# Thefefe/orbit

Hardware: AMD Instinct MI355X
Metric: meshlets_culled_per_sec (higher is better)
Workload: dtype f32

## Files before the change

### bindings/rust/orbit_hip.rs

```rust
#![allow(non_camel_case_types, dead_code)]
use std::ffi::{c_char, c_void};

#[repr(C)]
pub struct OrbitCtx { _private: [u8; 0] }
#[repr(C)]
pub struct OrbitMeshletStream { _private: [u8; 0] }

#[repr(C)] #[derive(Clone, Copy, Default)]
pub struct OrbitCaps {
    pub max_entities: u32, pub max_dispatches: u32, pub max_draws: u32, pub max_lights: u32,
    pub max_clusters: u32, pub dispatch_size: u32, pub max_views: u32, pub validate_streams: u32, pub cull_path: u32,
    pub arith_profile: u32,
}

#[repr(C)]
pub struct OrbitClusterFrame {
    pub push: *const c_void, pub info: *const c_void, pub depth: *const f32, pub lights: *const c_void,
    pub tile_depth_slice_mask: *mut u32, pub depth_bounds: *mut c_void, pub unique_cluster_buffer: *mut c_void,
    pub light_index_buffer: *mut c_void, pub cluster_offset_image: *mut u32,
    pub index_capacity: u32, pub light_index_capacity: u32,
}
#[repr(C)]
pub struct OrbitFrameLate {
    pub pyramids: *const c_void, pub late_views: *const c_void, pub cascade_views: *const c_void,
// ... 162 lines not shown
                                   draw_first: u32, draw_count: u32, stream: *mut c_void) -> i32;
    pub fn orbit_meshlet_cull(ctx: *mut OrbitCtx, cull_info: *const c_void, bufs: *const OrbitMeshletCullBufs,
                              stream: *mut c_void) -> i32;
    pub fn orbit_depth_pyramid_desc(screen_w: u32, screen_h: u32, desc: *mut OrbitDepthPyramidDesc) -> i32;
    pub fn orbit_depth_pyramid_desc_from_mip0(mip0_w: u32, mip0_h: u32, desc: *mut OrbitDepthPyramidDesc) -> i32;
    pub fn orbit_ctx_profile(ctx: *mut OrbitCtx, enable: i32) -> i32;
    pub fn orbit_ctx_profile_reserve(ctx: *mut OrbitCtx, pairs: u32, stream: *mut c_void) -> i32;
    pub fn orbit_ctx_profile_read(ctx: *mut OrbitCtx, avg_ms: *mut f32, launches: *mut u32) -> i32;
    pub fn orbit_cull_views(ctx: *mut OrbitCtx, views: *const OrbitCullView, count: u32, stream: *mut c_void) -> i32;
    pub fn orbit_depth_reduce(ctx: *mut OrbitCtx, depth: *const f32, screen_w: u32, screen_h: u32,
                              pyramid: *mut f32, stream: *mut c_void) -> i32;
    pub fn orbit_depth_reduce_multi(ctx: *mut OrbitCtx, items: *const OrbitDepthReduceItem, count: u32,
                                    stream: *mut c_void) -> i32;
    pub fn orbit_cluster_mark(ctx: *mut OrbitCtx, push: *const c_void, depth: *const f32, masks: *mut u32,
                              bounds: *mut c_void, stream: *mut c_void) -> i32;
    pub fn orbit_cluster_compact(ctx: *mut OrbitCtx, cluster_count: *const [u32; 3], masks: *const u32,
                                 unique: *mut c_void, index_capacity: u32, stream: *mut c_void) -> i32;
    pub fn orbit_cluster_assign(ctx: *mut OrbitCtx, info: *const c_void, unique: *const c_void, bounds: *const c_void,
                                lights: *const c_void, light_index_buffer: *mut c_void, light_index_capacity: u32,
                                cluster_offset_image: *mut u32, stream: *mut c_void) -> i32;
    pub fn orbit_meshlet_task_cull(ctx: *mut OrbitCtx, cull_info: *const c_void, bufs: *const c_void,
                                   task_records: *mut c_void, stream: *mut c_void) -> i32;
    pub fn orbit_compute_clusters(ctx: *mut OrbitCtx, push: *const c_void, info: *const c_void, depth: *const f32,
                                  lights: *const c_void, masks: *mut u32, bounds: *mut c_void, unique: *mut c_void,
                                  index_capacity: u32, light_index_buffer: *mut c_void, light_index_capacity: u32,
                                  cluster_offset_image: *mut u32, stream: *mut c_void) -> i32;
    pub fn orbit_shard_range(entity_draw_count: u32, rank: u32, world: u32, begin: *mut u32, end: *mut u32);
    pub fn orbit_gather_visible(ctx: *mut OrbitCtx, nccl_comm: *mut c_void, rank: u32, world: u32,
                                local_draw_buffer: *const c_void, out_draw_buffer: *mut c_void, out_capacity: u32,
                                stream: *mut c_void) -> i32;
    pub fn orbit_meshlet_cull_visible_records(ctx: *mut OrbitCtx, cull_info: *const c_void, bufs: *const c_void,
                                              record_buffer: *mut c_void, record_capacity: u32,
                                              stream: *mut c_void) -> i32;
    pub fn orbit_expand_visible_records(ctx: *mut OrbitCtx, record_buffer: *const c_void, meshlet_buffer: *const c_void,
                                        draw_commands_buffer: *mut c_void, draw_capacity: u32,
                                        stream: *mut c_void) -> i32;
    pub fn orbit_meshlet_stream_create(ctx: *mut OrbitCtx, first_meshlet: u64, capacity: u64,
                                       out_stream: *mut *mut OrbitMeshletStream) -> i32;
    pub fn orbit_meshlet_stream_update(ctx: *mut OrbitCtx, ms: *mut OrbitMeshletStream, meshlet_buffer: *const c_void,
                                       first: u64, count: u64, stream: *mut c_void) -> i32;
    pub fn orbit_meshlet_stream_set_materials(ctx: *mut OrbitCtx, ms: *mut OrbitMeshletStream, material_buffer: *const c_void,
                                              material_count: u32, stream: *mut c_void) -> i32;
    pub fn orbit_meshlet_stream_validate(ctx: *mut OrbitCtx, ms: *mut OrbitMeshletStream, meshlet_buffer: *const c_void,
                                         material_buffer: *const c_void, stream: *mut c_void) -> i32;
    pub fn orbit_meshlet_stream_destroy(ms: *mut OrbitMeshletStream) -> i32;
    pub fn orbit_meshlet_stream_update_meshes(ctx: *mut OrbitCtx, ms: *mut OrbitMeshletStream, mesh_info_buffer: *const c_void,
                                              first_mesh: u32, count: u32, stream: *mut c_void) -> i32;
    pub fn orbit_ctx_mesh_side_culls(ctx: *const OrbitCtx) -> u64;
    pub fn orbit_ctx_bind_meshlet_stream(ctx: *mut OrbitCtx, ms: *mut OrbitMeshletStream) -> i32;
    pub fn orbit_ctx_fused_culls(ctx: *const OrbitCtx) -> u64;
    pub fn orbit_frame_late(ctx: *mut OrbitCtx, frame: *const OrbitFrameLate, stream: *mut c_void) -> i32;
    pub fn orbit_ctx_meshlet_stream_culls(ctx: *const OrbitCtx) -> u64;
    pub fn orbit_ctx_meshlet_class_culls(ctx: *const OrbitCtx) -> u64;
    pub fn orbit_p2p_alloc(ctx: *mut OrbitCtx, bytes: u64, out_ptr: *mut *mut c_void, out_handle: *mut [u8; 64]) -> i32;
    pub fn orbit_p2p_free(ctx: *mut OrbitCtx, ptr: *mut c_void) -> i32;
    pub fn orbit_p2p_open(ctx: *mut OrbitCtx, handle: *const [u8; 64], out_peer_ptr: *mut *mut c_void) -> i32;
    pub fn orbit_p2p_close(ctx: *mut OrbitCtx, peer_ptr: *mut c_void) -> i32;
    pub fn orbit_meshlet_cull_records_and_commands(ctx: *mut OrbitCtx, cull_info: *const c_void,
                                                   bufs: *const OrbitMeshletCullBufs, record_buffer: *mut c_void,
                                                   record_capacity: u32, stream: *mut c_void) -> i32;
    pub fn orbit_exchange_list(ctx: *mut OrbitCtx, local_list: *const c_void, rank: u32, world: u32,
                               out_buffers: *const *mut c_void, ctrl_buffers: *const *mut c_void, out_capacity: u32,
                               header_bytes: u32, stride: u32, stream: *mut c_void) -> i32;
    pub fn orbit_cull_shard(ctx: *mut OrbitCtx, cull_info: *const c_void, entity_bufs: *const OrbitEntityCullBufs,
                            draw_first: u32, draw_count: u32, meshlet_bufs: *const OrbitMeshletCullBufs,
                            record_buffer: *mut c_void, record_capacity: u32, with_commands: u32,
                            stream: *mut c_void) -> i32;
    pub fn orbit_ctx_shard_culls(ctx: *const OrbitCtx) -> u64;
    pub fn orbit_allgather_list(ctx: *mut OrbitCtx, nccl_comm: *mut c_void, rank: u32, world: u32,
                                local_list: *const c_void, segment_capacity: u32, segments: *mut c_void,
                                out_list: *mut c_void, out_capacity: u32, header_bytes: u32, stride: u32,
                                stream: *mut c_void) -> i32;
    pub fn orbit_compact_segments(ctx: *mut OrbitCtx, segments: *const c_void, world: u32, segment_capacity: u32,
                                  out_list: *mut c_void, out_capacity: u32, header_bytes: u32, stride: u32,
                                  stream: *mut c_void) -> i32;
    pub fn orbit_scene_update_entities(ctx: *mut OrbitCtx, transforms: *const OrbitEntityTransform,
                                       instance_indices: *const u32, count: u32, entity_data: *mut c_void,
                                       entity_capacity: u32, stream: *mut c_void) -> i32;
    pub fn orbit_scene_update(ctx: *mut OrbitCtx, update: *const OrbitSceneUpdate, stream: *mut c_void) -> i32;
    pub fn orbit_cull_stats(ctx: *mut OrbitCtx, cull_info: *const c_void, ebufs: *const OrbitEntityCullBufs,
                            entity_draw_count: u32, mbufs: *const OrbitMeshletCullBufs, stats: *mut OrbitCullStats,
                            stream: *mut c_void) -> i32;
    pub fn orbit_cluster_stats(ctx: *mut OrbitCtx, push: *const c_void, info: *const c_void, depth: *const f32,
                               lights: *const c_void, stats: *mut OrbitClusterStats, stream: *mut c_void) -> i32;
    pub fn orbit_meshlet_bounds(ctx: *mut OrbitCtx, job: *const OrbitMeshletBoundsJob, stream: *mut c_void) -> i32;
    pub fn orbit_mesh_bounds(ctx: *mut OrbitCtx, ranges: *const OrbitMeshBoundsRange, range_count: u32,
                             vertices: *const c_void, vertex_count: u64, vertex_stride: u32, position_offset: u32,
                             mesh_infos: *mut c_void, mesh_capacity: u32, stream: *mut c_void) -> i32;
    pub fn orbit_raster_depth(ctx: *mut OrbitCtx, job: *const OrbitRasterDepth, stream: *mut c_void) -> i32;
    pub fn orbit_raster_visibility(ctx: *mut OrbitCtx, job: *const OrbitRasterVisibility, stream: *mut c_void) -> i32;
    pub fn orbit_visibility_resolve(ctx: *mut OrbitCtx, job: *const OrbitVisibilityResolve, stream: *mut c_void) -> i32;
}

pub fn check(ctx: *const OrbitCtx, rc: i32) {
    if rc != 0 {
        let msg = unsafe { std::ffi::CStr::from_ptr(orbit_last_error(ctx)) }.to_string_lossy().into_owned();
        panic!("orbit_hip error {rc}: {msg}");
    }
}
```

### include/orbit_abi_ext.h

```cpp
#ifndef ORBIT_ABI_EXT_H
#define ORBIT_ABI_EXT_H

#include "orbit_abi.h"

#ifdef __cplusplus
extern "C" {
#endif

#define ORBIT_VISIBLE_HEADER 8u
typedef struct OrbitVisibleRecord {
    uint32_t entity_index;
    uint32_t meshlet_offset;
    uint32_t mask;
} OrbitVisibleRecord;
ORBIT_STATIC_ASSERT(sizeof(OrbitVisibleRecord) == 12, "visible record is 12 B");

int32_t orbit_meshlet_task_cull(OrbitCtx *ctx, const OrbitGpuCullInfo *cull_info,
                                const OrbitMeshletCullBufs *bufs,
                                OrbitMeshTaskRecord *task_records, void *stream);

typedef struct OrbitCullView {
    const OrbitGpuCullInfo *cull_info;
    OrbitEntityCullBufs entity;
    OrbitMeshletCullBufs meshlet;
    uint32_t entity_draw_count;
    uint32_t skip_meshlet_stage;
} OrbitCullView;
#define ORBIT_MAX_CULL_VIEWS 8
int32_t orbit_cull_views(OrbitCtx *ctx, const OrbitCullView *views, uint32_t count, void *stream);
uint64_t orbit_ctx_fused_culls(const OrbitCtx *ctx);

typedef struct OrbitMeshletStream OrbitMeshletStream;
int32_t orbit_meshlet_stream_create(OrbitCtx *ctx, uint64_t first_meshlet, uint64_t capacity,
                                    OrbitMeshletStream **out_stream);
int32_t orbit_meshlet_stream_update(OrbitCtx *ctx, OrbitMeshletStream *ms, const void *meshlet_buffer,
                                    uint64_t first, uint64_t count, void *stream);
int32_t orbit_meshlet_stream_set_materials(OrbitCtx *ctx, OrbitMeshletStream *ms, const void *material_buffer,
                                           uint32_t material_count, void *stream);
int32_t orbit_meshlet_stream_validate(OrbitCtx *ctx, OrbitMeshletStream *ms, const void *meshlet_buffer,
                                      const void *material_buffer, void *stream);
int32_t orbit_meshlet_stream_update_meshes(OrbitCtx *ctx, OrbitMeshletStream *ms, const void *mesh_info_buffer,
                                           uint32_t first_mesh, uint32_t count, void *stream);
uint64_t orbit_ctx_mesh_side_culls(const OrbitCtx *ctx);
int32_t orbit_meshlet_stream_destroy(OrbitMeshletStream *ms);
int32_t orbit_ctx_bind_meshlet_stream(OrbitCtx *ctx, OrbitMeshletStream *ms);
uint64_t orbit_ctx_meshlet_stream_culls(const OrbitCtx *ctx);
uint64_t orbit_ctx_meshlet_class_culls(const OrbitCtx *ctx);

typedef struct OrbitDepthReduceItem {
    const float *depth;
    uint32_t screen_width, screen_height;
    uint32_t depth_row_pitch;
    uint32_t _pad;
    float *pyramid;
    const OrbitDepthPyramidLevel *levels;
} OrbitDepthReduceItem;
ORBIT_STATIC_ASSERT(sizeof(OrbitDepthReduceItem) == 40, "depth-reduce item is 40 B");
#define ORBIT_MAX_PYRAMID_BATCH 8
int32_t orbit_depth_reduce_multi(OrbitCtx *ctx, const OrbitDepthReduceItem *items, uint32_t count, void *stream);

typedef struct OrbitClusterFrame {
    const OrbitMarkActivePush *push;
    const OrbitClusterCullInfo *info;
    const float *depth;
    const OrbitLightData *lights;
    uint32_t *tile_depth_slice_mask;
    OrbitClusterDepthBounds *depth_bounds;
    void *unique_cluster_buffer;
    void *light_index_buffer;
    uint32_t *cluster_offset_image;
    uint32_t index_capacity;
    uint32_t light_index_capacity;
} OrbitClusterFrame;
ORBIT_STATIC_ASSERT(sizeof(OrbitClusterFrame) == 80, "cluster frame block is 80 B");
typedef struct OrbitFrameLate {
    const OrbitDepthReduceItem *pyramids;
    const OrbitCullView *late_views;
    const OrbitCullView *cascade_views;
    const OrbitClusterFrame *clusters;
    uint32_t pyramid_count, late_view_count, cascade_view_count, _pad;
} OrbitFrameLate;
ORBIT_STATIC_ASSERT(sizeof(OrbitFrameLate) == 48, "frame-late descriptor is 48 B");
int32_t orbit_frame_late(OrbitCtx *ctx, const OrbitFrameLate *frame, void *stream);

int32_t orbit_ctx_profile(OrbitCtx *ctx, int32_t enable);
int32_t orbit_ctx_profile_reserve(OrbitCtx *ctx, uint32_t pairs, void *stream);
int32_t orbit_ctx_profile_read(OrbitCtx *ctx, float *avg_ms, uint32_t *launches);

int32_t orbit_meshlet_cull_visible_records(OrbitCtx *ctx, const OrbitGpuCullInfo *cull_info,
                                           const OrbitMeshletCullBufs *bufs, void *record_buffer,
                                           uint32_t record_capacity, void *stream);
int32_t orbit_expand_visible_records(OrbitCtx *ctx, const void *record_buffer, const void *meshlet_buffer,
                                     void *draw_commands_buffer, uint32_t draw_capacity, void *stream);
int32_t orbit_meshlet_cull_records_and_commands(OrbitCtx *ctx, const OrbitGpuCullInfo *cull_info,
                                                const OrbitMeshletCullBufs *bufs, void *record_buffer,
                                                uint32_t record_capacity, void *stream);
int32_t orbit_cull_shard(OrbitCtx *ctx, const OrbitGpuCullInfo *cull_info, const OrbitEntityCullBufs *entity_bufs,
                         uint32_t draw_first, uint32_t draw_count, const OrbitMeshletCullBufs *meshlet_bufs,
                         void *record_buffer, uint32_t record_capacity, uint32_t with_commands, void *stream);
uint64_t orbit_ctx_shard_culls(const OrbitCtx *ctx);
// ... 228 lines not shown
```

### orbit_amd/_lib.py

```python
import ctypes as C
import os

_HERE = os.path.dirname(os.path.abspath(__file__))
LIB_PATH = os.path.join(_HERE, "liborbit_cull.so")

OK, E_INVALID, E_PLANES, E_CAPACITY, E_HIP, E_NO_DEVICE, E_TIMEOUT, E_MISSING, E_COMM, E_RANGE, E_STALE = (
    0, -1, -2, -3, -4, -5, -6, -7, -8, -9, -10)
ERROR_NAMES = {
    E_INVALID: "ORBIT_E_INVALID", E_PLANES: "ORBIT_E_PLANES", E_CAPACITY: "ORBIT_E_CAPACITY", E_HIP: "ORBIT_E_HIP",
    E_NO_DEVICE: "ORBIT_E_NO_DEVICE", E_TIMEOUT: "ORBIT_E_TIMEOUT", E_MISSING: "ORBIT_E_MISSING",
    E_COMM: "ORBIT_E_COMM", E_RANGE: "ORBIT_E_RANGE", E_STALE: "ORBIT_E_STALE",
}

MAX_PYRAMID_MIPS = 16


class OrbitError(RuntimeError):
    def __init__(self, code, message):
        super().__init__(f"{ERROR_NAMES.get(code, code)}: {message}")
        self.code = code


class Caps(C.Structure):
    _fields_ = [("max_entities", C.c_uint32), ("max_dispatches", C.c_uint32), ("max_draws", C.c_uint32),
# ... 104 lines not shown
                                                            C.c_void_p, C.c_uint32, C.c_void_p]),
    "orbit_exchange_list": (C.c_int32, [C.c_void_p, C.c_void_p, C.c_uint32, C.c_uint32, C.POINTER(C.c_void_p),
                                        C.POINTER(C.c_void_p), C.c_uint32, C.c_uint32, C.c_uint32, C.c_void_p]),
    "orbit_ctx_fused_culls": (C.c_uint64, [C.c_void_p]),
    "orbit_frame_late": (C.c_int32, [C.c_void_p, C.POINTER(FrameLate), C.c_void_p]),
    "orbit_default_caps": (None, [C.POINTER(Caps)]),
    "orbit_ctx_create": (C.c_int32, [C.c_int32, C.POINTER(Caps), C.POINTER(C.c_void_p)]),
    "orbit_ctx_destroy": (C.c_int32, [C.c_void_p]),
    "orbit_last_error": (C.c_char_p, [C.c_void_p]),
    "orbit_ctx_status": (C.c_int32, [C.c_void_p, C.c_void_p, C.c_int32]),
    "orbit_entity_cull": (C.c_int32, [C.c_void_p, C.c_void_p, C.POINTER(EntityCullBufs), C.c_uint32, C.c_void_p]),
    "orbit_entity_cull_range": (C.c_int32, [C.c_void_p, C.c_void_p, C.POINTER(EntityCullBufs), C.c_uint32,
                                            C.c_uint32, C.c_void_p]),
    "orbit_meshlet_cull": (C.c_int32, [C.c_void_p, C.c_void_p, C.POINTER(MeshletCullBufs), C.c_void_p]),
    "orbit_meshlet_task_cull": (C.c_int32, [C.c_void_p, C.c_void_p, C.POINTER(MeshletCullBufs), C.c_void_p, C.c_void_p]),
    "orbit_depth_pyramid_desc": (C.c_int32, [C.c_uint32, C.c_uint32, C.POINTER(DepthPyramidDesc)]),
    "orbit_cull_views": (C.c_int32, [C.c_void_p, C.POINTER(CullView), C.c_uint32, C.c_void_p]),
    "orbit_depth_reduce_multi": (C.c_int32, [C.c_void_p, C.POINTER(DepthReduceItem), C.c_uint32, C.c_void_p]),
    "orbit_depth_pyramid_desc_from_mip0": (C.c_int32, [C.c_uint32, C.c_uint32, C.POINTER(DepthPyramidDesc)]),
    "orbit_depth_reduce": (C.c_int32, [C.c_void_p, C.c_void_p, C.c_uint32, C.c_uint32, C.c_void_p, C.c_void_p]),
    "orbit_cluster_mark": (C.c_int32, [C.c_void_p, C.c_void_p, C.c_void_p, C.c_void_p, C.c_void_p, C.c_void_p]),
    "orbit_cluster_compact": (C.c_int32, [C.c_void_p, C.POINTER(C.c_uint32 * 3), C.c_void_p, C.c_void_p, C.c_uint32,
                                          C.c_void_p]),
    "orbit_cluster_assign": (C.c_int32, [C.c_void_p, C.c_void_p, C.c_void_p, C.c_void_p, C.c_void_p, C.c_void_p,
                                         C.c_uint32, C.c_void_p, C.c_void_p]),
    "orbit_compute_clusters": (C.c_int32, [C.c_void_p, C.c_void_p, C.c_void_p, C.c_void_p, C.c_void_p, C.c_void_p,
                                           C.c_void_p, C.c_void_p, C.c_uint32, C.c_void_p, C.c_uint32, C.c_void_p,
                                           C.c_void_p]),
    "orbit_ctx_profile": (C.c_int32, [C.c_void_p, C.c_int32]),
    "orbit_ctx_profile_reserve": (C.c_int32, [C.c_void_p, C.c_uint32, C.c_void_p]),
    "orbit_ctx_profile_read": (C.c_int32, [C.c_void_p, C.POINTER(C.c_float), C.POINTER(C.c_uint32)]),
    "orbit_shard_range": (None, [C.c_uint32, C.c_uint32, C.c_uint32, C.POINTER(C.c_uint32), C.POINTER(C.c_uint32)]),
    "orbit_gather_visible": (C.c_int32, [C.c_void_p, C.c_void_p, C.c_uint32, C.c_uint32, C.c_void_p, C.c_void_p,
                                         C.c_uint32, C.c_void_p]),
    "orbit_meshlet_cull_visible_records": (C.c_int32, [C.c_void_p, C.c_void_p, C.POINTER(MeshletCullBufs), C.c_void_p,
                                                       C.c_uint32, C.c_void_p]),
    "orbit_expand_visible_records": (C.c_int32, [C.c_void_p, C.c_void_p, C.c_void_p, C.c_void_p, C.c_uint32,
                                                 C.c_void_p]),
    "orbit_p2p_alloc": (C.c_int32, [C.c_void_p, C.c_uint64, C.POINTER(C.c_void_p), C.c_void_p]),
    "orbit_p2p_free": (C.c_int32, [C.c_void_p, C.c_void_p]),
    "orbit_p2p_open": (C.c_int32, [C.c_void_p, C.c_void_p, C.POINTER(C.c_void_p)]),
    "orbit_p2p_close": (C.c_int32, [C.c_void_p, C.c_void_p]),
    "orbit_meshlet_stream_create": (C.c_int32, [C.c_void_p, C.c_uint64, C.c_uint64, C.POINTER(C.c_void_p)]),
    "orbit_meshlet_stream_update": (C.c_int32, [C.c_void_p, C.c_void_p, C.c_void_p, C.c_uint64, C.c_uint64,
                                                C.c_void_p]),
    "orbit_meshlet_stream_set_materials": (C.c_int32, [C.c_void_p, C.c_void_p, C.c_void_p, C.c_uint32, C.c_void_p]),
    "orbit_meshlet_stream_validate": (C.c_int32, [C.c_void_p, C.c_void_p, C.c_void_p, C.c_void_p, C.c_void_p]),
    "orbit_meshlet_stream_destroy": (C.c_int32, [C.c_void_p]),
    "orbit_meshlet_stream_update_meshes": (C.c_int32, [C.c_void_p, C.c_void_p, C.c_void_p, C.c_uint32, C.c_uint32, C.c_void_p]),
    "orbit_ctx_mesh_side_culls": (C.c_uint64, [C.c_void_p]),
    "orbit_ctx_bind_meshlet_stream": (C.c_int32, [C.c_void_p, C.c_void_p]),
    "orbit_ctx_meshlet_stream_culls": (C.c_uint64, [C.c_void_p]),
    "orbit_ctx_meshlet_class_culls": (C.c_uint64, [C.c_void_p]),
    "orbit_cull_shard": (C.c_int32, [C.c_void_p, C.c_void_p, C.POINTER(EntityCullBufs), C.c_uint32, C.c_uint32,
                                     C.POINTER(MeshletCullBufs), C.c_void_p, C.c_uint32, C.c_uint32, C.c_void_p]),
    "orbit_ctx_shard_culls": (C.c_uint64, [C.c_void_p]),
    "orbit_allgather_list": (C.c_int32, [C.c_void_p, C.c_void_p, C.c_uint32, C.c_uint32, C.c_void_p, C.c_uint32,
                                         C.c_void_p, C.c_void_p, C.c_uint32, C.c_uint32, C.c_uint32, C.c_void_p]),
    "orbit_compact_segments": (C.c_int32, [C.c_void_p, C.c_void_p, C.c_uint32, C.c_uint32, C.c_void_p, C.c_uint32,
                                           C.c_uint32, C.c_uint32, C.c_void_p]),
    "orbit_scene_update_entities": (C.c_int32, [C.c_void_p, C.c_void_p, C.c_void_p, C.c_uint32, C.c_void_p, C.c_uint32,
                                                C.c_void_p]),
    "orbit_scene_update": (C.c_int32, [C.c_void_p, C.POINTER(SceneUpdate), C.c_void_p]),
    "orbit_cull_stats": (C.c_int32, [C.c_void_p, C.c_void_p, C.POINTER(EntityCullBufs), C.c_uint32,
                                     C.POINTER(MeshletCullBufs), C.c_void_p, C.c_void_p]),
    "orbit_cluster_stats": (C.c_int32, [C.c_void_p, C.c_void_p, C.c_void_p, C.c_void_p, C.c_void_p, C.c_void_p,
                                        C.c_void_p]),
    "orbit_meshlet_bounds": (C.c_int32, [C.c_void_p, C.POINTER(MeshletBoundsJob), C.c_void_p]),
    "orbit_mesh_bounds": (C.c_int32, [C.c_void_p, C.c_void_p, C.c_uint32, C.c_void_p, C.c_uint64, C.c_uint32, C.c_uint32,
                                      C.c_void_p, C.c_uint32, C.c_void_p]),
    "orbit_raster_depth": (C.c_int32, [C.c_void_p, C.POINTER(RasterDepth), C.c_void_p]),
    "orbit_raster_visibility": (C.c_int32, [C.c_void_p, C.POINTER(RasterVisibility), C.c_void_p]),
    "orbit_visibility_resolve": (C.c_int32, [C.c_void_p, C.POINTER(VisibilityResolve), C.c_void_p]),
}

_lib = None


def load_variant(path):
    import torch

    lib = C.CDLL(path)
    for name, (restype, argtypes) in SYMBOLS.items():
        if hasattr(lib, name):
            fn = getattr(lib, name)
            fn.restype = restype
            fn.argtypes = argtypes
    return lib


def load():
    global _lib
    if _lib is not None:
        return _lib
    if not os.path.exists(LIB_PATH):
        raise OSError(f"{LIB_PATH} is missing: build it with `make -C orbit_amd/csrc` or "
                      "`python -c 'import __graft_entry__ as g; g.build()'` (there is no fallback path)")
    try:
        import torch
    except ImportError:
        pass
    lib = C.CDLL(LIB_PATH)
    for name, (restype, argtypes) in SYMBOLS.items():
        fn = getattr(lib, name)
        fn.restype = restype
        fn.argtypes = argtypes
# ... 9 lines not shown
```

### orbit_amd/csrc/abi_ctx.hip

```cpp
#include <cstdarg>
#include <cstdio>
#include <cstdlib>

#include "abi_internal.h"

thread_local char g_err[512] = "no error";

int32_t fail(OrbitCtx *ctx, int32_t code, const char *fmt, ...) {
    char buf[512];
    va_list ap;
    va_start(ap, fmt);
    vsnprintf(buf, sizeof(buf), fmt, ap);
    va_end(ap);
    snprintf(g_err, sizeof(g_err), "%s", buf);
    if (ctx) snprintf(ctx->err, sizeof(ctx->err), "%s", buf);
    return code;
}

namespace {

size_t layout_arena(OrbitCtx *ctx, uintptr_t base, uint64_t md32) {
    const OrbitCaps &caps = ctx->caps;
    const size_t ent = align_up((size_t)caps.max_entities, 256);
    const size_t mtiles = ((size_t)md32 + kTileRecords - 1) / kTileRecords + 1;
// ... 84 lines not shown
                    caps.max_dispatches, caps.dispatch_size, max_dispatch_capacity());
    if (caps.arith_profile > ORBIT_ARITH_CONTRACTED)
        return fail(nullptr, ORBIT_E_INVALID, "arith_profile %u (0 canonical, 1 contracted)", caps.arith_profile);
    if (caps.max_dispatches > max_dispatch_capacity())
        return fail(nullptr, ORBIT_E_CAPACITY, "caps.max_dispatches %u > %u (chunk-base table of the emit launch)",
                    caps.max_dispatches, max_dispatch_capacity());
    int ndev = 0;
    hipError_t e = hipGetDeviceCount(&ndev);
    if (e != hipSuccess || ndev <= 0 || device_id < 0 || device_id >= ndev)
        return fail(nullptr, ORBIT_E_NO_DEVICE, "no usable HIP device %d (count %d): %s; there is no CPU fallback",
                    device_id, ndev, e == hipSuccess ? "ok" : hipGetErrorString(e));
    hipDeviceProp_t prop;
    e = hipGetDeviceProperties(&prop, device_id);
    if (e != hipSuccess) return hip_fail(nullptr, e, "hipGetDeviceProperties");
    if (strncmp(prop.gcnArchName, "gfx950", 6) != 0)
        return fail(nullptr, ORBIT_E_NO_DEVICE, "device %d is %s; this library carries gfx950 code objects only",
                    device_id, prop.gcnArchName);
    e = hipSetDevice(device_id);
    if (e != hipSuccess) return hip_fail(nullptr, e, "hipSetDevice");
    if (caps.cull_path > 2u)
        return fail(nullptr, ORBIT_E_INVALID, "caps.cull_path %u (0 auto, 1 launch chain, 2 one-launch cull)", caps.cull_path);
    if (caps.max_views > ORBIT_MAX_CULL_VIEWS)
        return fail(nullptr, ORBIT_E_CAPACITY, "caps.max_views %u > %u", caps.max_views, (unsigned)ORBIT_MAX_CULL_VIEWS);

    OrbitCtx *ctx = new (std::nothrow) OrbitCtx();
    if (!ctx) return fail(nullptr, ORBIT_E_HIP, "out of host memory");
    ctx->device = device_id;
    ctx->num_cus = (uint32_t)prop.multiProcessorCount;
    for (uint32_t v = 0; v < kRasterVariants; v++)
        with_raster_variant((RasterVariant)v, [&](auto variant) {
            ctx->raster_blocks[v] = ctx->num_cus * raster_depth_blocks_per_cu<variant.value>();
            ctx->visibility_blocks[v] = ctx->num_cus * raster_visibility_blocks_per_cu<variant.value>();
        });
    ctx->caps = caps;
    ctx->rec_shift = rec_shift;

    ctx->arena_bytes = layout_arena(ctx, 0, md32);
    e = hipMalloc((void **)&ctx->arena, ctx->arena_bytes);
    if (e != hipSuccess) {
        delete ctx;
        return hip_fail(nullptr, e, "hipMalloc(scratch arena)");
    }
    e = memset_now(ctx->arena, 0, ctx->arena_bytes);
    if (e != hipSuccess) {
        (void)hipFree(ctx->arena);
        delete ctx;
        return hip_fail(nullptr, e, "hipMemset(scratch arena)");
    }
    (void)layout_arena(ctx, (uintptr_t)ctx->arena, md32);
#ifdef ORBIT_TRIAGE
    const char *dbg = getenv("ORBIT_SP_DEBUG");
    ctx->debug_flags = dbg ? (uint32_t)atoi(dbg) : 0u;
#endif
    snprintf(ctx->err, sizeof(ctx->err), "no error");
    const OrbitCaps child_caps = view_child_caps(caps);
    for (uint32_t v = 1; v < caps.max_views; v++) {
        OrbitCtx *child = nullptr;
        const int32_t rc = orbit_ctx_create(device_id, &child_caps, &child);
        if (rc != ORBIT_OK) {
            (void)orbit_ctx_destroy(ctx);
            return rc;
        }
        ctx->view_ctx.push_back(child);
    }
    *out_ctx = ctx;
    return ORBIT_OK;
}

int32_t orbit_ctx_destroy(OrbitCtx *ctx) {
    if (!ctx) return ORBIT_OK;
    (void)hipSetDevice(ctx->device);
    (void)hipDeviceSynchronize();
    for (hipEvent_t ev : ctx->prof_events) (void)hipEventDestroy(ev);
    for (hipEvent_t ev : ctx->side_event)
        if (ev) (void)hipEventDestroy(ev);
    for (hipStream_t st : ctx->side_stream)
        if (st) (void)hipStreamDestroy(st);
    for (OrbitCtx *child : ctx->view_ctx) (void)orbit_ctx_destroy(child);
    if (ctx->meshlet_stream) ctx->meshlet_stream->bindings.fetch_sub(1);
    if (ctx->arena) (void)hipFree(ctx->arena);
    delete ctx;
    return ORBIT_OK;
}

int32_t orbit_ctx_status(OrbitCtx *ctx, void *stream, int32_t sync) {
    if (!ctx) return fail(nullptr, ORBIT_E_INVALID, "ctx is NULL");
    std::lock_guard<std::mutex> lock(ctx->mu);
    hipStream_t s = (hipStream_t)stream;
    if (sync) {
        hipError_t e = hipStreamSynchronize(s);
        if (e != hipSuccess) return hip_fail(ctx, e, "hipStreamSynchronize");
    }
    int32_t v = 0;
    hipError_t e = hipMemcpy(&v, ctx->status, 4, hipMemcpyDeviceToHost);
    if (e != hipSuccess) return hip_fail(ctx, e, "hipMemcpy(status)");
    for (OrbitCtx *child : ctx->view_ctx) {
        int32_t cv = 0;
        e = hipMemcpy(&cv, child->status, 4, hipMemcpyDeviceToHost);
        if (e != hipSuccess) return hip_fail(ctx, e, "hipMemcpy(status)");
        if (cv != 0) {
            (void)memset_now(child->status, 0, 4);
            if (v == 0) v = cv;
        }
    }
    if (v != 0) {
        e = memset_now(ctx->status, 0, 4);
// ... 117 lines not shown
```

### orbit_amd/csrc/abi_cull.hip

```cpp
#include "abi_internal.h"

namespace {

int32_t check_cull_info(OrbitCtx *ctx, const OrbitGpuCullInfo *ci) {
    if (!ci) return fail(ctx, ORBIT_E_INVALID, "cull_info is NULL");
    if (ci->cull_plane_count > ORBIT_MAX_CULL_PLANES)
        return fail(ctx, ORBIT_E_PLANES, "cull_plane_count %u > %d", ci->cull_plane_count, ORBIT_MAX_CULL_PLANES);
    if (ci->projection_type > 1) return fail(ctx, ORBIT_E_INVALID, "projection_type %u", ci->projection_type);
    if (ci->occlusion_pass > 2) return fail(ctx, ORBIT_E_INVALID, "occlusion_pass %u", ci->occlusion_pass);
    return ORBIT_OK;
}

MeshSideView mesh_side_for(OrbitMeshletStream *ms, const void *mesh_info_buffer, bool count = true) {
    if (!ms) return MeshSideView{nullptr, 0u};
    std::lock_guard<std::mutex> lock(ms->mu);
    if (ms->mesh_side == nullptr || ms->mesh_source != mesh_info_buffer || ms->mesh_hi == 0u) return MeshSideView{nullptr, 0u};
    if (count) ms->mesh_side_culls++;
    return MeshSideView{ms->mesh_side, ms->mesh_hi};
}

PyramidView make_pyramid_view(const float *texels, const uint32_t size[2],
                              const OrbitDepthPyramidLevel *levels = nullptr) {
    PyramidView v;
    v.texels = texels;
// ... 131 lines not shown
        ok = ok && zero(pl[4][0]) && zero(pl[4][1]);
        const float v[6] = {pl[0][0], pl[0][2], pl[2][1], pl[2][2], pl[4][2], pl[4][3]};
        for (float f : v) ok = ok && fin(f);
        p.std_planes = ok ? 1u : 0u;
        for (int k = 0; k < 6; k++) p.stdp[k] = ok ? v[k] : 0.0f;
    }
    p.task_records = task ? (OrbitMeshTaskRecord *)out.buffer : nullptr;
    p.also_commands = out.also_commands ? (uint8_t *)b->draw_commands_buffer : nullptr;
    p.also_commands_capacity = out.also_commands ? b->draw_capacity : 0u;
    p.tile_counts = scratch->m_tile_counts;
    p.tile_masks = scratch->m_tile_masks;
    p.tile_payload = scratch->m_tile_payload;
    p.tile_base = scratch->m_tile_base;
    p.chunk_sums = scratch->m_chunk_sums;
    p.total = scratch->m_total;
    p.tickets = scratch->m_tickets;
    p.list_sync = scratch->m_list_sync;
    p.debug_flags = scratch->debug_flags;
    p.debug_cycles = scratch->debug_cycles;
    p.scan_patience = ctx->scan_patience;
    p.zero_page = scratch->zero_page;
    p.status = scratch->status;
    return ORBIT_OK;
}

SplitRecordsParams split_params_for(const OrbitCtx *ctx, const OrbitCtx *scratch, const OrbitMeshletCullBufs *b) {
    SplitRecordsParams sp;
    sp.src = (const uint8_t *)b->meshlet_dispatch_buffer;
    sp.dst = scratch->m_split;
    sp.src_capacity = b->dispatch_capacity;
    sp.rec_shift = ctx->rec_shift;
    return sp;
}

int32_t profile_pair(OrbitCtx *ctx, hipEvent_t &ev0, hipEvent_t &ev1) {
    ev0 = ev1 = nullptr;
    if (!ctx->profiling || (ctx->prof_calls++ % ctx->profiling) != 0) return ORBIT_OK;
    if (ctx->prof_used + 2 > ctx->prof_events.size()) {
        for (int i = 0; i < 2; i++) {
            hipEvent_t ev;
            if (hipEventCreate(&ev) != hipSuccess) return fail(ctx, ORBIT_E_HIP, "hipEventCreate");
            ctx->prof_events.push_back(ev);
        }
    }
    ev0 = ctx->prof_events[ctx->prof_used];
    ev1 = ctx->prof_events[ctx->prof_used + 1];
    ctx->prof_used += 2;
    return ORBIT_OK;
}

int32_t validate_stream(OrbitCtx *ctx, const MeshletCullParams &p, hipStream_t s) {
    if (!p.ms.sphere || !ctx->caps.validate_streams) return ORBIT_OK;
    const hipError_t e = launch_meshlet_stream_validate(p.meshlets, p.ms, p.ms.cls0 ? p.materials : nullptr,
                                                        ctx->meshlet_stream->material_count, ctx->status, s);
    return e == hipSuccess ? ORBIT_OK : hip_fail(ctx, e, "launch meshlet_stream_validate");
}

void count_stream_cull(OrbitCtx *ctx, const MeshletCullParams &p) {
    if (p.ms.sphere && p.ci.occlusion_pass != 1) {
        ctx->stream_culls++;
        if (p.ms.cls0) ctx->class_culls++;
    }
}

int32_t entity_cull_impl(OrbitCtx *ctx, const OrbitGpuCullInfo *ci, const OrbitEntityCullBufs *b, uint32_t draw_first,
                         uint32_t entity_draw_count, bool exact_range, void *stream) {
    if (!ctx) return fail(nullptr, ORBIT_E_INVALID, "ctx is NULL");
    std::lock_guard<std::mutex> lock(ctx->mu);
    EntityCullParams p;
    int32_t rc = entity_cull_params(ctx, ctx, ci, b, draw_first, entity_draw_count, exact_range, p);
    if (rc == ORBIT_OK) rc = validate_mesh_side(ctx, p, (hipStream_t)stream);
    if (rc) return rc;
    const hipError_t e = launch_entity_cull(p, entity_draw_count, ctx->num_cus, (hipStream_t)stream);
    if (e != hipSuccess) return hip_fail(ctx, e, "launch entity_cull");
    return ORBIT_OK;
}

int32_t meshlet_cull_impl(OrbitCtx *ctx, const OrbitGpuCullInfo *ci, const OrbitMeshletCullBufs *b,
                          const MeshletCullOut &out, void *stream) {
    if (!ctx) return fail(nullptr, ORBIT_E_INVALID, "ctx is NULL");
    std::lock_guard<std::mutex> lock(ctx->mu);
    const hipStream_t s = (hipStream_t)stream;
    MeshletCullParams p;
    hipEvent_t ev0, ev1;
    int32_t rc = meshlet_cull_params(ctx, ctx, ci, b, out, p);
    if (rc == ORBIT_OK) rc = profile_pair(ctx, ev0, ev1);
    if (rc == ORBIT_OK && ci->occlusion_pass != 1) rc = validate_stream(ctx, p, s);
    if (rc) return rc;
    hipError_t e = hipSuccess;
    if (ctx->rec_shift > 5u) e = launch_split_records(split_params_for(ctx, ctx, b), s);
    if (e != hipSuccess) return hip_fail(ctx, e, "launch split_records");
    e = launch_meshlet_cull(p, ctx->num_cus, s, ev0, ev1);
    if (e != hipSuccess) return hip_fail(ctx, e, "launch meshlet_cull");
    count_stream_cull(ctx, p);
    return ORBIT_OK;
}

FusedCullParams fused_params(const EntityCullParams &ep, const MeshletCullParams &mp, const OrbitCtx *scratch,
                             uint32_t chunks) {
    FusedCullParams f{};
    f.m = mp;
    f.entity_draw_buffer = ep.entity_draw_buffer;
    f.mesh_infos = ep.mesh_infos;
    f.mesh_side = ep.mesh_side;
    f.visibility = ep.visibility;
    f.e_pyr = ep.pyr;
    f.draw_first = ep.draw_first;
    f.draw_limit = ep.draw_limit;
    f.e_dispatch_capacity = ep.dispatch_capacity;
    f.ne_chunks = chunks;
    f.e_total = ep.total;
    f.sync = scratch->f_sync;
    f.ent_flags = scratch->f_ent_flags;
    f.tile_flags = scratch->f_tile_flags;
    return f;
}

OrbitCtx *scratch_of(OrbitCtx *ctx, uint32_t k) { return k == 0 ? ctx : ctx->view_ctx[k - 1]; }

}

int32_t prepare_cull_views(OrbitCtx *ctx, const OrbitCullView *views, uint32_t count, uint32_t scratch_base,
                           PreparedCullViews &pc) {
    if (!views || count == 0) return fail(ctx, ORBIT_E_MISSING, "cull_views: no views");
    if (count > ORBIT_MAX_CULL_VIEWS || scratch_base + count > ORBIT_MAX_CULL_VIEWS)
        return fail(ctx, ORBIT_E_CAPACITY, "cull_views: %u views (max %u)", scratch_base + count, (unsigned)ORBIT_MAX_CULL_VIEWS);
    hipError_t e = hipSetDevice(ctx->device);
    if (e != hipSuccess) return hip_fail(ctx, e, "hipSetDevice");
    while (ctx->view_ctx.size() + 1 < scratch_base + count) {
        OrbitCtx *child = nullptr;
        const OrbitCaps child_caps = view_child_caps(ctx->caps);
        const int32_t rc = orbit_ctx_create(ctx->device, &child_caps, &child);
        if (rc != ORBIT_OK) return fail(ctx, rc, "cull_views: scratch for view %zu: %s", ctx->view_ctx.size() + 1, g_err);
        ctx->view_ctx.push_back(child);
    }
    pc.count = count;
    for (uint32_t i = 0; i < count; i++) {
        const OrbitCullView &v = views[i];
        OrbitCtx *scratch = scratch_of(ctx, scratch_base + i);
        int32_t rc = entity_cull_params(ctx, scratch, v.cull_info, &v.entity, 0u, v.entity_draw_count, false, pc.ev.v[i]);
        if (rc == ORBIT_OK && !v.skip_meshlet_stage) {
            rc = meshlet_cull_params(ctx, scratch, v.cull_info, &v.meshlet, MeshletCullOut{}, pc.mv.v[pc.n_mesh]);
            if (rc == ORBIT_OK && ctx->rec_shift > 5u) pc.sv.v[pc.n_mesh] = split_params_for(ctx, scratch, &v.meshlet);
            if (rc == ORBIT_OK && v.meshlet.meshlet_dispatch_buffer != v.entity.meshlet_dispatch_buffer)
                rc = fail(ctx, ORBIT_E_INVALID, "view %u: the meshlet stage must read the entity stage's dispatch buffer", i);
            pc.n_mesh++;
        }
// ... 209 lines not shown
```

### orbit_amd/csrc/abi_internal.h

```cpp
#pragma once
#include <hip/hip_runtime.h>

#include <atomic>
#include <cstdint>
#include <cstring>
#include <mutex>
#include <new>
#include <vector>

#include "kernels.h"

using namespace orbit;

#pragma GCC visibility push(hidden)

struct OrbitMeshletStream {
    int device = 0;
    uint64_t first = 0, capacity = 0;
    uint4 *sphere = nullptr;
    uint32_t *cone = nullptr;
    uint16_t *mat = nullptr;
    uint32_t *cmd = nullptr;
    uint16_t *cnt = nullptr;
    uint32_t *link = nullptr, *cls0 = nullptr, *cls1 = nullptr;
    uint2 *base32 = nullptr;
    std::mutex mu;
    const void *source = nullptr;
    uint64_t valid_lo = 0, valid_hi = 0;
    const void *materials = nullptr;
    uint32_t material_count = 0;
    uint32_t *d_other = nullptr, *h_other = nullptr;
    hipEvent_t other_event = nullptr;
    bool other_pending = false;
    bool other_recorded = false;
    std::atomic<int> bindings{0};
    MeshSide *mesh_side = nullptr;
    uint32_t mesh_capacity = 0, mesh_hi = 0;
    const void *mesh_source = nullptr;
    uint64_t mesh_side_culls = 0;
};

struct OrbitCtx {
    int device = 0;
    uint32_t num_cus = 0;
    OrbitCaps caps{};
    std::mutex mu;
    uint8_t *arena = nullptr;
    size_t arena_bytes = 0;
    OrbitMeshletDispatch *e_proto = nullptr;
    uint32_t *e_block_sums = nullptr, *e_total = nullptr;
    Payload *m_tile_payload = nullptr;
    uint32_t *m_tile_masks = nullptr, *m_chunk_sums = nullptr;
    uint32_t *m_tile_counts = nullptr, *m_tile_base = nullptr, *m_total = nullptr;
    uint32_t *s_block_sums = nullptr;
    uint32_t raster_blocks[kRasterVariants] = {};
    uint32_t visibility_blocks[kRasterVariants] = {};
    float *b_mesh_slices = nullptr;
    uint32_t *x_block_pop = nullptr;
    uint32_t *c_chunk = nullptr;
    size_t c_chunk_words = 0;
    float4 *a_view_lights = nullptr, *a_coarse_lights = nullptr;
    uint32_t *a_light_flags = nullptr, *a_counts = nullptr, *a_block_sums = nullptr, *a_block_base = nullptr,
             *a_total = nullptr, *a_coarse = nullptr, *a_coarse_counts = nullptr, *a_hit_cache = nullptr;
    float *a_aabb = nullptr, *a_group_box = nullptr;
    uint32_t *a_group_order = nullptr;
    uint32_t a_coarse_seg = 0;
    uint32_t *m_tickets = nullptr, *m_list_sync = nullptr, *f_done = nullptr;
    uint32_t *f_sync = nullptr, *f_ent_flags = nullptr, *f_tile_flags = nullptr;
    uint32_t *d_tickets = nullptr;
    uint8_t *m_split = nullptr;
    uint32_t rec_shift = 5;
    uint64_t fused_culls = 0;
    uint64_t shard_culls = 0;
    uint32_t *g_counts = nullptr;
    int32_t *status = nullptr;
    uint32_t debug_flags = 0;
    uint32_t scan_patience = 256;
    unsigned long long *debug_cycles = nullptr;
    void *zero_page = nullptr;
    uint32_t profiling = 0;
    uint32_t prof_calls = 0;
    std::vector<hipEvent_t> prof_events;
    size_t prof_used = 0;
    std::vector<OrbitCtx *> view_ctx;
    hipStream_t side_stream[2] = {nullptr, nullptr};
    hipEvent_t side_event[3] = {nullptr, nullptr, nullptr};
    OrbitMeshletStream *meshlet_stream = nullptr;
    uint64_t stream_culls = 0;
    uint64_t class_culls = 0;
    char err[512] = {0};
};

constexpr uint32_t kExpandBlocks = 65536;

constexpr uint32_t kMeshBoundsSlots = 1024;

extern thread_local char g_err[512];

int32_t fail(OrbitCtx *ctx, int32_t code, const char *fmt, ...);

inline int32_t hip_fail(OrbitCtx *ctx, hipError_t e, const char *what) {
    return fail(ctx, ORBIT_E_HIP, "%s: %s", what, hipGetErrorString(e));
}

inline size_t align_up(size_t v, size_t a) { return (v + a - 1) / a * a; }

inline hipError_t memset_now(void *ptr, int value, size_t bytes) {
    hipError_t e = hipMemset(ptr, value, bytes);
    if (e == hipSuccess) e = hipStreamSynchronize(nullptr);
    return e;
}

inline uint32_t mip_levels_from_size(uint32_t max_size) {
    uint32_t l = 0;
    while ((max_size >> (l + 1)) != 0) l++;
    return l + 1;
}

inline OrbitCaps view_child_caps(OrbitCaps child_caps) {
    child_caps.max_views = 0, child_caps.max_clusters = 0, child_caps.max_lights = 0;
    return child_caps;
}

inline MeshletStreamView stream_arrays(const OrbitMeshletStream *ms, uint64_t lo, uint64_t hi) {
    MeshletStreamView v{};
    v.sphere = ms->sphere - ms->first;
    v.cone = ms->cone - ms->first;
    v.mat = ms->mat - ms->first;
    v.cmd = ms->cmd - 3u * ms->first;
    v.cnt = ms->cnt - ms->first;
    v.link = ms->link - (ms->first >> 5);
    v.base32 = ms->base32 - (ms->first >> 5);
    v.cls0 = ms->cls0 - (ms->first >> 5);
    v.cls1 = ms->cls1 - (ms->first >> 5);
    v.first = (uint32_t)lo;
    v.count = (uint32_t)(hi - lo);
    return v;
}

inline MeshletStreamView stream_view_for(OrbitMeshletStream *ms, const void *meshlet_buffer, const void *material_buffer) {
    if (!ms) return MeshletStreamView{};
    std::lock_guard<std::mutex> lock(ms->mu);
    if (ms->source == nullptr || ms->source != meshlet_buffer || ms->valid_hi == ms->valid_lo) return MeshletStreamView{};
    MeshletStreamView v = stream_arrays(ms, ms->valid_lo, ms->valid_hi);
    bool classes = ms->materials != nullptr && ms->materials == material_buffer;
    if (classes && ms->other_pending && ms->other_recorded && hipEventQuery(ms->other_event) == hipSuccess)
        ms->other_pending = false;
    if (classes && (ms->other_pending || *ms->h_other != 0u)) classes = false;
    if (!classes) v.cls0 = v.cls1 = nullptr;
    return v;
}

struct PreparedCullViews {
    EntityCullViews ev{};
    MeshletCullViews mv{};
    FusedCullViews fv{};
    SplitRecordsViews sv{};
    uint32_t draws[ORBIT_MAX_CULL_VIEWS] = {};
    uint32_t count = 0, n_mesh = 0, max_draws = 0;
    bool fused = false;
};

int32_t prepare_cull_views(OrbitCtx *ctx, const OrbitCullView *views, uint32_t count, uint32_t scratch_base,
                           PreparedCullViews &pc);
int32_t launch_prepared_cull_views(OrbitCtx *ctx, const PreparedCullViews &pc, hipStream_t s);

#pragma GCC visibility pop
```

### orbit_amd/csrc/abi_stream.hip

```cpp
#include "abi_internal.h"

namespace {

constexpr uint32_t kMeshSideMinCapacity = 1u << 20;

hipError_t read_back_class_flag(OrbitMeshletStream *ms, hipStream_t s) {
    ms->other_pending = true;
    ms->other_recorded = false;
    hipStreamCaptureStatus cs = hipStreamCaptureStatusNone;
    if (hipStreamIsCapturing(s, &cs) != hipSuccess || cs != hipStreamCaptureStatusNone) return hipSuccess;
    hipError_t e = hipMemcpyAsync(ms->h_other, ms->d_other, sizeof(uint32_t), hipMemcpyDeviceToHost, s);
    if (e == hipSuccess) e = hipEventRecord(ms->other_event, s);
    if (e == hipSuccess) ms->other_recorded = true;
    return e;
}

int32_t check_stream(OrbitCtx *ctx, const OrbitMeshletStream *ms, const char *who, bool takes_buffer = false, const void *buffer = nullptr) {
    if (takes_buffer ? !ms || !buffer : !ms)
        return fail(ctx, ORBIT_E_MISSING, takes_buffer ? "%s: NULL argument" : "%s: stream is NULL", who);
    if (ms->device != ctx->device) return fail(ctx, ORBIT_E_INVALID, "%s: stream lives on device %d", who, ms->device);
    return ORBIT_OK;
}

}

extern "C" {

int32_t orbit_meshlet_stream_create(OrbitCtx *ctx, uint64_t first_meshlet, uint64_t capacity,
                                    OrbitMeshletStream **out_stream) {
    if (!ctx) return fail(nullptr, ORBIT_E_INVALID, "ctx is NULL");
    std::lock_guard<std::mutex> lock(ctx->mu);
    if (!out_stream) return fail(ctx, ORBIT_E_MISSING, "meshlet_stream_create: out_stream is NULL");
    *out_stream = nullptr;
    if (capacity == 0 || capacity > (1ull << 27) || first_meshlet + capacity > 0xFFFFFFFFull)
        return fail(ctx, ORBIT_E_INVALID, "meshlet_stream_create: range [%llu, +%llu) (at most 2^27 meshlets per stream)",
                    (unsigned long long)first_meshlet, (unsigned long long)capacity);
    hipError_t e = hipSetDevice(ctx->device);
    if (e != hipSuccess) return hip_fail(ctx, e, "hipSetDevice");
    OrbitMeshletStream *ms = new (std::nothrow) OrbitMeshletStream();
    if (!ms) return fail(ctx, ORBIT_E_HIP, "out of host memory");
    ms->device = ctx->device;
    ms->first = first_meshlet;
    ms->capacity = capacity;
    const size_t bit_words = (size_t)(((first_meshlet + capacity + 31u) >> 5) - (first_meshlet >> 5)) + 2u;
    struct {
        void **p;
        size_t bytes;
        int fill;
    } arrays[] = {{(void **)&ms->sphere, capacity * sizeof(uint4), 0},
                  {(void **)&ms->cone, capacity * sizeof(uint32_t), 0},
                  {(void **)&ms->mat, capacity * sizeof(uint16_t) + 256u, 0},
                  {(void **)&ms->cmd, capacity * 12u, 0},
                  {(void **)&ms->cnt, capacity * sizeof(uint16_t) + 256u, 0},
                  {(void **)&ms->link, bit_words * sizeof(uint32_t), 0},
                  {(void **)&ms->base32, bit_words * sizeof(uint2), 0},
                  {(void **)&ms->cls0, bit_words * sizeof(uint32_t), 0xFF},
                  {(void **)&ms->cls1, bit_words * sizeof(uint32_t), 0xFF}};
    for (auto &a : arrays) {
        if (e == hipSuccess) e = hipMalloc(a.p, a.bytes);
        if (e == hipSuccess) e = hipMemset(*a.p, a.fill, a.bytes);
    }
    if (e == hipSuccess) e = hipMalloc((void **)&ms->d_other, 256);
    if (e == hipSuccess) e = memset_now(ms->d_other, 0, 256);
    if (e == hipSuccess) e = hipHostMalloc((void **)&ms->h_other, sizeof(uint32_t), hipHostMallocDefault);
    if (e == hipSuccess) *ms->h_other = 0u;
    if (e == hipSuccess) e = hipEventCreateWithFlags(&ms->other_event, hipEventDisableTiming);
    if (e != hipSuccess) {
        orbit_meshlet_stream_destroy(ms);
        return hip_fail(ctx, e, "meshlet_stream_create: hipMalloc (36.65 B per meshlet)");
    }
    *out_stream = ms;
    return ORBIT_OK;
}

int32_t orbit_meshlet_stream_update(OrbitCtx *ctx, OrbitMeshletStream *ms, const void *meshlet_buffer, uint64_t first,
                                    uint64_t count, void *stream) {
    if (!ctx) return fail(nullptr, ORBIT_E_INVALID, "ctx is NULL");
    std::lock_guard<std::mutex> lock(ctx->mu);
    if (const int32_t rc = check_stream(ctx, ms, "meshlet_stream_update", true, meshlet_buffer)) return rc;
    if (first < ms->first || count > ms->capacity || first - ms->first > ms->capacity - count)
        return fail(ctx, ORBIT_E_CAPACITY, "meshlet_stream_update: [%llu, +%llu) outside the stream's [%llu, +%llu)",
                    (unsigned long long)first, (unsigned long long)count, (unsigned long long)ms->first,
                    (unsigned long long)ms->capacity);
    std::lock_guard<std::mutex> slock(ms->mu);
    const bool same = ms->source == meshlet_buffer && ms->valid_hi > ms->valid_lo;
    const uint64_t lo = same ? (first < ms->valid_lo ? first : ms->valid_lo) : first;
    const uint64_t hi = same ? (first + count > ms->valid_hi ? first + count : ms->valid_hi) : first + count;
    MeshletStreamView v = stream_arrays(ms, same ? ms->valid_lo : first, same ? ms->valid_hi : first + count);
    if (v.first > first) v.count += v.first - (uint32_t)first, v.first = (uint32_t)first;
    if ((uint64_t)v.first + v.count < first + count) v.count = (uint32_t)(first + count - v.first);
    hipError_t e = launch_meshlet_stream_build((const OrbitMeshlet *)meshlet_buffer, first, count, v,
                                               (const OrbitMaterialData *)ms->materials, ms->material_count, ms->d_other,
                                               (hipStream_t)stream);
    if (e != hipSuccess) return hip_fail(ctx, e, "launch meshlet_stream_build");
    if (ms->materials != nullptr && count != 0) {
        e = read_back_class_flag(ms, (hipStream_t)stream);
        if (e != hipSuccess) return hip_fail(ctx, e, "meshlet_stream_update: class flag read-back");
    }
    if (count != 0) {
        ms->source = meshlet_buffer;
        ms->valid_lo = lo;
        ms->valid_hi = hi;
    }
    return ORBIT_OK;
}

int32_t orbit_meshlet_stream_set_materials(OrbitCtx *ctx, OrbitMeshletStream *ms, const void *material_buffer,
                                           uint32_t material_count, void *stream) {
    if (!ctx) return fail(nullptr, ORBIT_E_INVALID, "ctx is NULL");
    std::unique_lock<std::mutex> lock(ctx->mu);
    if (const int32_t rc = check_stream(ctx, ms, "meshlet_stream_set_materials")) return rc;
    if (material_buffer && material_count == 0)
        return fail(ctx, ORBIT_E_INVALID, "meshlet_stream_set_materials: material_count is 0");
    std::unique_lock<std::mutex> slock(ms->mu);
    ms->other_pending = true;
    ms->other_recorded = false;
    hipError_t e = hipMemsetAsync(ms->d_other, 0, sizeof(uint32_t), (hipStream_t)stream);
    if (e == hipSuccess)
        e = launch_meshlet_stream_classes(stream_arrays(ms, ms->first, ms->first + ms->capacity),
                                          (const OrbitMaterialData *)material_buffer, material_buffer ? material_count : 0u,
                                          ms->d_other, (hipStream_t)stream);
    if (e == hipSuccess) e = read_back_class_flag(ms, (hipStream_t)stream);
    if (e != hipSuccess) return hip_fail(ctx, e, "launch meshlet_stream_classes");
    ms->materials = material_buffer;
    ms->material_count = material_buffer ? material_count : 0u;
    const bool wait = ms->other_recorded;
    hipEvent_t ev = ms->other_event;
    slock.unlock();
    lock.unlock();
    if (wait) {
        e = hipEventSynchronize(ev);
        if (e != hipSuccess) {
            lock.lock();
            return hip_fail(ctx, e, "hipEventSynchronize(alpha-class flag)");
        }
    }
    return ORBIT_OK;
}

int32_t orbit_meshlet_stream_update_meshes(OrbitCtx *ctx, OrbitMeshletStream *ms, const void *mesh_info_buffer,
                                           uint32_t first_mesh, uint32_t count, void *stream) {
    if (!ctx) return fail(nullptr, ORBIT_E_INVALID, "ctx is NULL");
    std::lock_guard<std::mutex> lock(ctx->mu);
    if (const int32_t rc = check_stream(ctx, ms, "meshlet_stream_update_meshes")) return rc;
    std::lock_guard<std::mutex> slock(ms->mu);
    if (!mesh_info_buffer) {
        ms->mesh_source = nullptr;
// ... 9 lines not shown
        if (e == hipSuccess) e = memset_now(ms->mesh_side, 0, (size_t)cap * sizeof(MeshSide));
        if (e != hipSuccess) {
            (void)hipFree(ms->mesh_side);
            ms->mesh_side = nullptr;
            return hip_fail(ctx, e, "meshlet_stream_update_meshes: hipMalloc (32 B per mesh)");
        }
        ms->mesh_capacity = cap;
    }
    if (first_mesh + count > ms->mesh_capacity)
        return fail(ctx, ORBIT_E_CAPACITY, "meshlet_stream_update_meshes: meshes [%u, +%u) beyond the table's %u", first_mesh,
                    count, ms->mesh_capacity);
    if (ms->mesh_source != mesh_info_buffer && ms->mesh_hi != 0u) {
        e = hipMemsetAsync(ms->mesh_side, 0, (size_t)ms->mesh_hi * sizeof(MeshSide), (hipStream_t)stream);
        if (e != hipSuccess) return hip_fail(ctx, e, "meshlet_stream_update_meshes: hipMemsetAsync");
        ms->mesh_hi = 0u;
    }
    e = launch_mesh_side_build((const OrbitMeshInfo *)mesh_info_buffer, first_mesh, count, ms->mesh_side, (hipStream_t)stream);
    if (e != hipSuccess) return hip_fail(ctx, e, "launch mesh_side_build");
    if (count != 0u) {
        ms->mesh_source = mesh_info_buffer;
        if (first_mesh + count > ms->mesh_hi) ms->mesh_hi = first_mesh + count;
    }
    return ORBIT_OK;
}

uint64_t orbit_ctx_mesh_side_culls(const OrbitCtx *ctx) {
    if (!ctx || !ctx->meshlet_stream) return 0;
    std::lock_guard<std::mutex> lock(ctx->meshlet_stream->mu);
    return ctx->meshlet_stream->mesh_side_culls;
}

int32_t orbit_meshlet_stream_validate(OrbitCtx *ctx, OrbitMeshletStream *ms, const void *meshlet_buffer,
                                      const void *material_buffer, void *stream) {
    if (!ctx) return fail(nullptr, ORBIT_E_INVALID, "ctx is NULL");
    std::lock_guard<std::mutex> lock(ctx->mu);
    if (const int32_t rc = check_stream(ctx, ms, "meshlet_stream_validate", true, meshlet_buffer)) return rc;
    {
        std::lock_guard<std::mutex> slock(ms->mu);
        if (ms->mesh_side != nullptr && ms->mesh_source != nullptr && ms->mesh_hi != 0u) {
            const hipError_t me = launch_mesh_side_validate((const OrbitMeshInfo *)ms->mesh_source, 0u, ms->mesh_hi, ms->mesh_side,
                                                            ctx->status, (hipStream_t)stream);
            if (me != hipSuccess) return hip_fail(ctx, me, "launch mesh_side_validate");
        }
    }
    MeshletStreamView v = stream_view_for(ms, meshlet_buffer, nullptr);
    if (!v.sphere) return ORBIT_OK;
    const bool classes = material_buffer != nullptr && ms->materials == material_buffer;
    if (classes) {
        const MeshletStreamView all = stream_arrays(ms, ms->first, ms->first + ms->capacity);
        v.cls0 = all.cls0, v.cls1 = all.cls1;
    }
    const hipError_t e = launch_meshlet_stream_validate((const OrbitMeshlet *)meshlet_buffer, v,
                                                        classes ? (const OrbitMaterialData *)material_buffer : nullptr,
                                                        ms->material_count, ctx->status, (hipStream_t)stream);
    if (e != hipSuccess) return hip_fail(ctx, e, "launch meshlet_stream_validate");
    return ORBIT_OK;
}

int32_t orbit_meshlet_stream_destroy(OrbitMeshletStream *ms) {
    if (!ms) return ORBIT_OK;
    if (ms->bindings.load() > 0)
        return fail(nullptr, ORBIT_E_INVALID, "meshlet_stream_destroy: the stream is still bound to %d context(s)",
                    ms->bindings.load());
    (void)hipFree(ms->sphere);
    (void)hipFree(ms->cone);
    (void)hipFree(ms->mat);
    (void)hipFree(ms->cmd);
    (void)hipFree(ms->cnt);
    (void)hipFree(ms->link);
    (void)hipFree(ms->base32);
    (void)hipFree(ms->cls0);
    (void)hipFree(ms->cls1);
    (void)hipFree(ms->d_other);
    (void)hipFree(ms->mesh_side);
    if (ms->h_other) (void)hipHostFree(ms->h_other);
    if (ms->other_event) (void)hipEventDestroy(ms->other_event);
    delete ms;
    return ORBIT_OK;
}

int32_t orbit_ctx_bind_meshlet_stream(OrbitCtx *ctx, OrbitMeshletStream *ms) {
    if (!ctx) return fail(nullptr, ORBIT_E_INVALID, "ctx is NULL");
    std::lock_guard<std::mutex> lock(ctx->mu);
    if (const int32_t rc = ms ? check_stream(ctx, ms, "bind_meshlet_stream") : ORBIT_OK) return rc;
    if (ms) ms->bindings.fetch_add(1);
    if (ctx->meshlet_stream) ctx->meshlet_stream->bindings.fetch_sub(1);
    ctx->meshlet_stream = ms;
    return ORBIT_OK;
}

uint64_t orbit_ctx_fused_culls(const OrbitCtx *ctx) { return ctx ? ctx->fused_culls : 0; }
uint64_t orbit_ctx_meshlet_stream_culls(const OrbitCtx *ctx) { return ctx ? ctx->stream_culls : 0; }
uint64_t orbit_ctx_meshlet_class_culls(const OrbitCtx *ctx) { return ctx ? ctx->class_culls : 0; }
uint64_t orbit_ctx_shard_culls(const OrbitCtx *ctx) { return ctx ? ctx->shard_culls : 0; }

}
```

### orbit_amd/csrc/kernels.h

```cpp
#pragma once
#include <hip/hip_runtime.h>
#include <stdint.h>
#include <type_traits>

#include "../../include/orbit_abi_ext.h"
#include "orbit_device.h"

namespace orbit {

constexpr uint32_t kTileRecords = 16;
constexpr uint32_t kTileRows = 8;
constexpr uint32_t kTicketPools = 8;
constexpr uint32_t kTicketStride = 64;
constexpr uint32_t kEmitTicketPools = 16;
constexpr uint32_t kListGroups = 32;
constexpr uint32_t kListSyncStride = 32;
constexpr uint32_t kListSyncWords = (kListGroups + 1) * kListSyncStride;

struct Payload {
    uint32_t y, z, w;
};

struct MeshSide {
    float sphere[4];
    uint32_t lod_count, lod0_offset, lod0_count, valid;
};
static_assert(sizeof(MeshSide) == 32, "MeshSide layout");
struct MeshSideView {
    const MeshSide *table;
    uint32_t count;
};

struct EntityCullParams {
    OrbitGpuCullInfo ci;
    const uint8_t *entity_draw_buffer;
    const OrbitMeshInfo *mesh_infos;
    MeshSideView mesh_side;
    uint8_t *dispatch_buffer;
    const OrbitEntityData *entities;
    uint32_t *visibility;
    PyramidView pyr;
    uint32_t draw_first;
    uint32_t draw_limit;
    uint32_t dispatch_capacity;
    uint32_t ne_chunks;
    uint32_t rec_shift;
    uint32_t arith;
    OrbitMeshletDispatch *proto;
    uint32_t *block_sums;
    uint32_t *sync;
    uint32_t *ent_flags;
    uint32_t *total;
    int32_t *status;
};

struct MeshletStreamView {
    const uint4 *sphere;
    const uint32_t *cone;
    const uint16_t *mat;
    const uint32_t *cmd;
    const uint16_t *cnt;
// ... 121 lines not shown
    PyramidView e_pyr;
    uint32_t draw_first, draw_limit;
    uint32_t e_dispatch_capacity;
    uint32_t ne_chunks;
    uint32_t *e_total;
    uint32_t *sync;
    uint32_t *ent_flags;
    uint32_t *tile_flags;
    uint32_t *done_flags;
};
struct FusedCullViews {
    FusedCullParams v[ORBIT_MAX_CULL_VIEWS];
};
hipError_t launch_cull_fused_views(const FusedCullViews &all, const uint32_t *entity_draw_counts, uint32_t n,
                                   uint32_t num_cus, hipStream_t s);
constexpr uint32_t kShardMaxChunks = 256;
constexpr uint32_t kShardDoneWords = 64, kShardDoneStride = 32;
hipError_t launch_shard_cull(const FusedCullParams &f, uint32_t num_cus, hipStream_t s);
hipError_t launch_meshlet_scan_emit(const MeshletCullParams &p, uint32_t num_cus, hipStream_t s);

hipError_t launch_entity_cull(const EntityCullParams &p, uint32_t entity_draw_count, uint32_t num_cus, hipStream_t s);
struct SplitRecordsParams {
    const uint8_t *src;
    uint8_t *dst;
    uint32_t src_capacity;
    uint32_t rec_shift;
};
struct SplitRecordsViews {
    SplitRecordsParams v[ORBIT_MAX_CULL_VIEWS];
};
hipError_t launch_split_records(const SplitRecordsParams &p, hipStream_t s);
hipError_t launch_split_records_views(const SplitRecordsViews &all, uint32_t n, hipStream_t s);

struct EntityCullViews {
    EntityCullParams v[ORBIT_MAX_CULL_VIEWS];
};
struct MeshletCullViews;
struct FusedCullViews;
struct ViewGroup;
#if !ORBIT_CONTRACT
hipError_t launch_entity_cull_contracted(const EntityCullParams &p, uint32_t entity_draw_count, uint32_t num_cus, hipStream_t s);
hipError_t launch_entity_cull_views_contracted(const EntityCullViews &all, uint32_t n, uint32_t max_entity_draw_count,
                                               uint32_t num_cus, hipStream_t s);
hipError_t launch_meshlet_eval_contracted(const MeshletCullParams &p, uint32_t num_cus, hipStream_t s);
hipError_t launch_meshlet_eval_views_contracted(const MeshletCullViews &all, const ViewGroup &g, uint32_t m, uint32_t pass,
                                                bool ortho, int src, uint32_t max_tiles, uint32_t num_cus, hipStream_t s);
hipError_t launch_shard_cull_contracted(const FusedCullParams &f, uint32_t num_cus, hipStream_t s);
hipError_t launch_cull_fused_views_contracted(const FusedCullViews &all, const uint32_t *entity_draw_counts, uint32_t n,
                                              uint32_t num_cus, hipStream_t s);
#endif
hipError_t launch_entity_cull_views(const EntityCullViews &all, uint32_t n, uint32_t max_entity_draw_count,
                                    uint32_t num_cus, hipStream_t s);
hipError_t launch_meshlet_cull(const MeshletCullParams &p, uint32_t num_cus, hipStream_t s,
                               hipEvent_t ev0 = nullptr, hipEvent_t ev1 = nullptr);
struct MeshletCullViews {
    MeshletCullParams v[ORBIT_MAX_CULL_VIEWS];
};
hipError_t launch_meshlet_cull_views(const MeshletCullViews &all, uint32_t n, uint32_t num_cus, hipStream_t s);
struct ViewGroup {
    uint8_t idx[ORBIT_MAX_CULL_VIEWS];
};
hipError_t launch_meshlet_eval(const MeshletCullParams &p, uint32_t num_cus, hipStream_t s);
hipError_t launch_meshlet_eval_views(const MeshletCullViews &all, const ViewGroup &g, uint32_t m, uint32_t pass,
                                     bool ortho, int src, uint32_t max_tiles, uint32_t num_cus, hipStream_t s);
hipError_t launch_meshlet_emit(const MeshletCullParams &p, bool stream, uint32_t num_cus, hipStream_t s);
hipError_t launch_meshlet_emit_views(const MeshletCullViews &all, const ViewGroup &g, uint32_t m, uint32_t n, bool stream,
                                     uint32_t max_tiles_all, uint32_t num_cus, hipStream_t s);
hipError_t launch_task_records(const MeshletCullParams &p, hipStream_t s);
uint32_t max_dispatch_capacity();
hipError_t launch_meshlet_stream_build(const OrbitMeshlet *meshlets, uint64_t first, uint64_t count,
                                       const MeshletStreamView &ms, const OrbitMaterialData *materials,
                                       uint32_t material_count, uint32_t *other, hipStream_t s);
hipError_t launch_meshlet_stream_validate(const OrbitMeshlet *meshlets, const MeshletStreamView &ms,
                                          const OrbitMaterialData *materials, uint32_t material_count, int32_t *status,
                                          hipStream_t s);
hipError_t launch_scene_update_entities(const OrbitEntityTransform *transforms, const uint32_t *instance_indices,
                                        uint32_t count, OrbitEntityData *entity_data, uint32_t entity_capacity,
                                        int32_t *status, hipStream_t s);
hipError_t launch_scene_update(const OrbitSceneUpdate &u, uint32_t *block_sums, int32_t *status, hipStream_t s);
hipError_t launch_meshlet_bounds(const OrbitMeshletBoundsJob &job, uint32_t num_cus, int32_t *status, hipStream_t s);
hipError_t launch_mesh_bounds(const OrbitMeshBoundsRange *ranges, uint32_t range_count, uint32_t slices,
                              const void *vertices, uint64_t vertex_count, uint32_t vertex_stride,
                              uint32_t position_offset, OrbitMeshInfo *mesh_infos, uint32_t mesh_capacity, float *scratch,
                              int32_t *status, hipStream_t s);
enum class RasterVariant : uint32_t { Plain, ClipNear, Wide };
constexpr uint32_t kRasterVariants = 3;
inline RasterVariant raster_variant(uint32_t flags) {
    return (flags & ORBIT_RASTER_WIDE_GUARD) ? RasterVariant::Wide : (flags & ORBIT_RASTER_CLIP_NEAR) ? RasterVariant::ClipNear : RasterVariant::Plain;
}
template <class F>
inline auto with_raster_variant(RasterVariant v, F f) {
    switch (v) {
    case RasterVariant::Wide: return f(std::integral_constant<RasterVariant, RasterVariant::Wide>{});
    case RasterVariant::ClipNear: return f(std::integral_constant<RasterVariant, RasterVariant::ClipNear>{});
    default: return f(std::integral_constant<RasterVariant, RasterVariant::Plain>{});
    }
}
template <RasterVariant V>
hipError_t launch_raster_depth(const OrbitRasterDepth &job, uint32_t resident_blocks, int32_t *status, hipStream_t s);
template <RasterVariant V>
hipError_t launch_raster_visibility(const OrbitRasterVisibility &job, uint32_t resident_blocks, int32_t *status, hipStream_t s);
template <RasterVariant V>
uint32_t raster_depth_blocks_per_cu();
template <RasterVariant V>
uint32_t raster_visibility_blocks_per_cu();
hipError_t launch_visibility_resolve(const OrbitVisibilityResolve &job, uint32_t num_cus, hipStream_t s);
struct CullStatsParams {
    EntityCullParams e;
    MeshletCullParams m;
    unsigned long long *stats;
};
hipError_t launch_cull_stats(const CullStatsParams &p, uint32_t num_cus, hipStream_t s);
#if !ORBIT_CONTRACT
hipError_t launch_cull_stats_contracted(const CullStatsParams &p, uint32_t num_cus, hipStream_t s);
#endif
struct ClusterStatsParams {
    OrbitMarkActivePush pc;
    OrbitClusterCullInfo info;
    const float *depth;
    const OrbitLightData *lights;
    unsigned long long *stats;
    unsigned long long samples;
    unsigned long long uncovered;
};
hipError_t launch_cluster_stats(const ClusterStatsParams &p, hipStream_t s);
hipError_t launch_mesh_side_build(const OrbitMeshInfo *mesh_infos, uint32_t first, uint32_t count, MeshSide *table, hipStream_t s);
hipError_t launch_mesh_side_validate(const OrbitMeshInfo *mesh_infos, uint32_t first, uint32_t count, const MeshSide *table,
                                     int32_t *status, hipStream_t s);
// ... 48 lines not shown
```

### orbit_amd/csrc/meshlet_common.h

```cpp
#pragma once
#include <type_traits>

#include "kernels.h"
#include "scan.h"

namespace orbit {

namespace {

constexpr uint32_t kPayloadCap = 128;

constexpr uint32_t kBufFlags = 0x00020000u;
constexpr uint32_t kNoOffset = 0xFFFFFF00u;

#ifndef ORBIT_EVAL_LOAD_AUX
#define ORBIT_EVAL_LOAD_AUX 2
#endif
#ifndef ORBIT_EMIT_CNT_AUX
#define ORBIT_EMIT_CNT_AUX 2
#endif
#ifndef ORBIT_EMIT_STORE_AUX
#define ORBIT_EMIT_STORE_AUX 0
#endif
struct StreamRsrc {
// ... 344 lines not shown
    const bool should_draw = should_draw_of(visible, abits, ((code >> 11) & 1u) != 0, true);
    const uint32_t word = (code >> 5) & 15u, bit = 1u << (code & 31u);
    if (visible) atomicOr(reinterpret_cast<uint32_t *>(L.vis_mask) + word, bit);
    if (should_draw) atomicOr(reinterpret_cast<uint32_t *>(L.draw_mask) + word, bit);
    const uint64_t dm = __ballot(should_draw);
    if (payload && should_draw) {
        const uint32_t rank = cs.total + lane_prefix(dm);
        if (rank < CAP)
            payload[rank] = make_payload(code & 31u, word, info);
    }
    cs.total += (uint32_t)__popcll(dm);
    cs.head = ring_wrap(cs.head + n);
    cs.count -= n;
}

template <int PROJ, int R, uint32_t N, bool CLS = false, uint32_t CAP = kPayloadCap>
__device__ __forceinline__ void row_eval_occ(const MeshletCullParams &p, WaveTileLds &L, const PlaneLds &P,
                                             const AlphaLds *A, CandLds<N> &C, int lane, const RowRegs<1> &t,
                                             CandState &cs, Payload *payload) {
    const uint32_t half = lane >> 5, ml = lane & 31;
    const uint32_t rid = 2 * R + half;
    const uint4 rec = L.r[rid].rec;
    const uint32_t abits = lane_alpha_bits<CLS>(p, L, A, rid, ml, t.b[0].w);
    const bool active = ml < rec.z;
    const bool visible_in_buffer = ((t.prev[0] >> ml) & 1u) != 0;
    Sphere s;
    s.x = s.y = s.z = s.r = 0.0f;
    bool cand = false;
    if (active) cand = eval_geometry<2, PROJ>(p, L, P, rid, t.a[0], t.b[0], visible_in_buffer, s, row_is_affine(L, R));
    const uint64_t mask = __ballot(cand);
    if (cand) {
        const uint32_t slot = ring_wrap(ring_wrap(cs.head + cs.count) + lane_prefix(mask));
        C.sphere[slot] = make_float4(s.x, s.y, s.z, __uint_as_float(t.a[0].w));
        C.info[slot] = make_uint4((uint32_t)(R * 64 + lane) | (abits << 9) | ((visible_in_buffer ? 1u : 0u) << 11),
                                  t.b[0].y, t.b[0].z, t.b[0].w);
    }
    cs.count += (uint32_t)__popcll(mask);
    if (cs.count >= kCandFlush) cand_flush<N, CAP>(p, L, C, lane, cs, min(cs.count, 64u), payload);
}

template <uint32_t N, uint32_t CAP = kPayloadCap>
__device__ __forceinline__ void tile_finish_occ(const MeshletCullParams &p, WaveTileLds &L, const CandLds<N> &C,
                                                int lane, CandState &cs, Payload *payload) {
    if (cs.count > 0) cand_flush<N, CAP>(p, L, C, lane, cs, cs.count, payload);
    __builtin_amdgcn_fence(__ATOMIC_RELEASE, "wavefront");
    __builtin_amdgcn_wave_barrier();
    __builtin_amdgcn_fence(__ATOMIC_ACQUIRE, "wavefront");
    if (lane < (int)kTileRecords) {
        const uint4 rec = L.r[lane].rec;
        uint32_t word = reinterpret_cast<const uint32_t *>(L.vis_mask)[lane];
        if (p.task_records && rec.z < 32u) word |= ~0u << rec.z;
        if (rec.z > 0) p.meshlet_visibility[rec.w] = word;
    }
}

__device__ __forceinline__ uint4 setup_load_rec(const MeshletCullParams &p, uint32_t tile, bool tile_valid,
                                                uint32_t nrec, int lane) {
    const OrbitMeshletDispatch *recs =
        reinterpret_cast<const OrbitMeshletDispatch *>(p.dispatch_buffer + ORBIT_DISPATCH_HEADER);
    const uint32_t rec_index = tile * kTileRecords + (uint32_t)(lane >> 2);
    const bool has = tile_valid && rec_index < nrec;
    const uint4 *src = has ? reinterpret_cast<const uint4 *>(recs + rec_index)
                           : reinterpret_cast<const uint4 *>(p.zero_page);
    return *src;
}

__device__ __forceinline__ float4 setup_load_mat(const MeshletCullParams &p, const uint4 &rec, int lane) {
#ifdef ORBIT_TRIAGE_NO_MAT
    return *reinterpret_cast<const float4 *>(p.zero_page);
#endif
    const float4 *src = rec.z != 0u ? reinterpret_cast<const float4 *>(p.entities[rec.x].model_matrix) + (lane & 3)
                                    : reinterpret_cast<const float4 *>(p.zero_page);
    return *src;
}

__device__ __forceinline__ uint32_t setup_load_cls(const MeshletCullParams &p, const uint4 &rec, int lane) {
    const uint32_t col = lane & 3;
    const uint32_t *plane = (col & 2u) ? p.ms.cls1 : p.ms.cls0;
    const uint32_t *src = (rec.z != 0u && p.ms.covers(rec.y)) ? plane + (rec.y >> 5) + (col & 1u)
                                                              : reinterpret_cast<const uint32_t *>(p.zero_page);
    return *src;
}

__device__ __forceinline__ void setup_write_cls(WaveTileLds &L, const uint32_t *sel, const uint4 &rec, uint32_t cls_word,
                                                int lane) {
    const uint32_t w0 = (uint32_t)__builtin_amdgcn_update_dpp(0, (int)cls_word, 0x00, 0xF, 0xF, false);
    const uint32_t w1 = (uint32_t)__builtin_amdgcn_update_dpp(0, (int)cls_word, 0x55, 0xF, 0xF, false);
    const uint32_t w2 = (uint32_t)__builtin_amdgcn_update_dpp(0, (int)cls_word, 0xAA, 0xF, 0xF, false);
    const uint32_t w3 = (uint32_t)__builtin_amdgcn_update_dpp(0, (int)cls_word, 0xFF, 0xF, 0xF, false);
    const uint32_t sh = rec.y & 31u;
    const uint32_t lo = __funnelshift_r(w0, w1, sh), hi = __funnelshift_r(w2, w3, sh);
    const uint32_t c0 = ~(hi | lo), c1 = lo & ~hi, c2 = hi & ~lo;
    const uint32_t exist = rec.z >= 32u ? ~0u : ~(~0u << (rec.z & 31u));
    if ((lane & 3) == 0)
        L.r[lane >> 2].amask = make_uint2(((c0 & sel[0]) | (c1 & sel[2]) | (c2 & sel[4])) & exist,
                                          ((c0 & sel[1]) | (c1 & sel[3]) | (c2 & sel[5])) & exist);
}

__device__ __forceinline__ void setup_write(const MeshletCullParams &p, WaveTileLds &L, const uint4 &rec,
                                            const float4 &mc, int lane, uint32_t prev_word = 0u) {
    const uint32_t rid = lane >> 2, col = lane & 3;
    float o[4];
    mat4_mul_col(p.ci.view_matrix, mc.x, mc.y, mc.z, mc.w, o);
    L.r[rid].mcol[col] = make_float4(o[0], o[1], o[2], o[3]);
    if (col == 3) L.r[rid].tzero = make_float4(o[0] * 0.0f, o[1] * 0.0f, o[2] * 0.0f, 0.0f);
    const float d = dot3(o[0], o[1], o[2], o[0], o[1], o[2]);
// ... 82 lines not shown
```

### orbit_amd/csrc/meshlet_cull.hip

```cpp
#include "kernels.h"

namespace orbit {

uint32_t max_dispatch_capacity() {
    const uint64_t cap = (uint64_t)kEmitChunkTable * kScanChunk * kTileRecords;
    return cap > 0xFFFFFFFFull ? 0xFFFFFFFFu : (uint32_t)cap;
}

namespace {

hipError_t scan_and_emit(const MeshletCullParams &p, uint32_t max_tiles, uint32_t num_cus, hipStream_t s) {
    const bool stream = p.ci.occlusion_pass != 1 && p.ms.sphere != nullptr;
    if (!stream) {
        const hipError_t e = launch_scan_chunks(p.tile_counts, p.tile_base, reinterpret_cast<const uint32_t *>(p.dispatch_buffer),
                                                kTileRecords, max_tiles, p.chunk_sums, s, p.tickets, kTicketPools * kTicketStride);
        if (e != hipSuccess) return e;
    }
    return launch_meshlet_emit(p, stream, num_cus, s);
}

}

hipError_t launch_meshlet_scan_emit(const MeshletCullParams &p, uint32_t num_cus, hipStream_t s) {
    const uint32_t max_tiles = (p.dispatch_capacity + kTileRecords - 1) / kTileRecords;
    if ((max_tiles + kScanChunk - 1) / kScanChunk > kEmitChunkTable) return hipErrorInvalidValue;
    return scan_and_emit(p, max_tiles, num_cus, s);
}

hipError_t launch_meshlet_cull(const MeshletCullParams &p, uint32_t num_cus, hipStream_t s, hipEvent_t ev0,
                               hipEvent_t ev1) {
    const uint32_t max_tiles = (p.dispatch_capacity + kTileRecords - 1) / kTileRecords;
    if ((max_tiles + kScanChunk - 1) / kScanChunk > kEmitChunkTable) return hipErrorInvalidValue;
    hipError_t e;
    if (ev0 && (e = hipEventRecord(ev0, s)) != hipSuccess) return e;
    if ((e = launch_meshlet_eval(p, num_cus, s)) != hipSuccess) return e;
    if (ev1 && (e = hipEventRecord(ev1, s)) != hipSuccess) return e;
    if (p.task_records) return launch_task_records(p, s);
    if (p.visible_list == 2u) {
        if (p.also_commands == nullptr) return hipSuccess;
        MeshletCullParams c = p;
        c.visible_list = 0u;
        c.draw_buffer = p.also_commands;
        c.draw_capacity = p.also_commands_capacity;
        return scan_and_emit(c, max_tiles, num_cus, s);
    }
    return scan_and_emit(p, max_tiles, num_cus, s);
}

hipError_t launch_meshlet_cull_views(const MeshletCullViews &all, uint32_t n, uint32_t num_cus, hipStream_t s) {
    if (n == 0) return hipSuccess;
    const MeshletCullParams *host = all.v;
    auto tiles_of = [&](uint32_t i) { return (host[i].dispatch_capacity + kTileRecords - 1) / kTileRecords; };
    uint32_t max_tiles_all = 0;
    for (uint32_t i = 0; i < n; i++) {
        if ((tiles_of(i) + kScanChunk - 1) / kScanChunk > kEmitChunkTable) return hipErrorInvalidValue;
        max_tiles_all = max(max_tiles_all, tiles_of(i));
    }
    auto source = [&](uint32_t i) -> int {
        if (host[i].ci.occlusion_pass == 1 || host[i].ms.sphere == nullptr) return 0;
        return host[i].ms.cls0 != nullptr ? 2 : 1;
    };
    bool done[ORBIT_MAX_CULL_VIEWS] = {};
    for (uint32_t i = 0; i < n; i++) {
        if (done[i]) continue;
        const uint32_t pass = host[i].ci.occlusion_pass, proj = host[i].ci.projection_type;
        const int src = source(i);
        ViewGroup g{};
        uint32_t m = 0, group_tiles = 0;
        for (uint32_t j = i; j < n; j++)
            if (!done[j] && host[j].ci.occlusion_pass == pass && host[j].ci.projection_type == proj && source(j) == src) {
                done[j] = true;
                g.idx[m++] = (uint8_t)j;
                group_tiles = max(group_tiles, tiles_of(j));
            }
        const hipError_t e = launch_meshlet_eval_views(all, g, m, pass, proj == 1, src, group_tiles, num_cus, s);
        if (e != hipSuccess) return e;
    }
    hipError_t e = hipSuccess;
    for (int stream = 0; stream < 2; stream++) {
        ViewGroup g{};
        uint32_t m = 0;
        for (uint32_t i = 0; i < n; i++)
            if ((source(i) != 0) == (stream != 0)) g.idx[m++] = (uint8_t)i;
        if (m == 0) continue;
        if (stream == 0) {
            ScanViews sv{};
            for (uint32_t k = 0; k < m; k++) {
                const uint32_t i = g.idx[k];
// ... 14 lines not shown
```

### orbit_amd/csrc/meshlet_eval.hip

```cpp
#include "entity_common.h"
#include "meshlet_common.h"

namespace orbit {

namespace {

constexpr int kEvWaves = 4;
constexpr int kEvWavesPerSimd = 4;
#ifndef ORBIT_EV_WPS0
#define ORBIT_EV_WPS0 5
#endif
constexpr int ev_waves_per_simd(int pass, bool stream) { return (pass == 0 && stream) ? ORBIT_EV_WPS0 : kEvWavesPerSimd; }


__device__ __forceinline__ void clear_chunk_sums(const MeshletCullParams &p) {
    if (blockIdx.x != 0) return;
    const uint32_t max_tiles = (p.dispatch_capacity + kTileRecords - 1) / kTileRecords;
    const uint32_t max_chunks = (max_tiles + kScanChunk - 1) / kScanChunk;
    for (uint32_t c = threadIdx.x; c < max_chunks; c += kEvWaves * 64) p.chunk_sums[c] = 0u;
    if (threadIdx.x < kEmitTicketPools) p.tickets[(kTicketPools + threadIdx.x) * kTicketStride] = 0u;
}

constexpr uint32_t kShardPatience = 256;

template <bool FUSED>
__device__ __forceinline__ uint4 eval_load_rec(const MeshletCullParams &p, uint32_t tile, bool tile_valid, uint32_t nrec, int lane) {
    if constexpr (FUSED) {
        const __amdgpu_buffer_rsrc_t R = rsrc_of(p.dispatch_buffer + ORBIT_DISPATCH_HEADER, nrec * 16u);
        const uint32_t rec_index = tile * kTileRecords + (uint32_t)(lane >> 2);
        const auto w = __builtin_amdgcn_raw_buffer_load_b128(R, (tile_valid && rec_index < nrec) ? rec_index * 16u : kNoOffset, 0, kSc1);
        return make_uint4(w[0], w[1], w[2], w[3]);
    } else {
        return setup_load_rec(p, tile, tile_valid, nrec, lane);
    }
}

template <int PASS, int PROJ, bool PROF, bool STREAM = false, bool CLS = false, bool LIST = false, bool FUSED = false>
__device__ __forceinline__ void meshlet_eval_body(const MeshletCullParams &p, const FusedCullParams *fp = nullptr) {
    static_assert(!FUSED || LIST, "the shard launch writes the record list");
    __shared__ std::conditional_t<FUSED, EntityChunksLds, uint32_t> ent_lds;
    __shared__ uint32_t s_word[2];
    __shared__ WaveTileLds lds[kEvWaves][3];
    __shared__ PlaneLds planes;
    __shared__ AlphaLds alpha_tab;
    __shared__ CandLds<(PASS == 2 ? kCandRing : 1u)> cand_ring[kEvWaves];
    const int lane = threadIdx.x & 63, wave = threadIdx.x >> 6;
#ifdef ORBIT_TRIAGE
    const unsigned long long wall_enter = wall_clock64();
    unsigned long long wall_chunks = 0;
#endif
    const bool occ2 = PASS == 2 && p.ci.meshlet_visibility_buffer != ORBIT_NONE;
    __shared__ uint32_t cls_sel[CLS ? 8 : 1];
    __shared__ uint32_t s_red[kEvWaves];
    uint32_t nrec_raw = 0;
    if constexpr (!FUSED) nrec_raw = *reinterpret_cast<const uint32_t *>(p.dispatch_buffer);
    const uint32_t stride = gridDim.x * kEvWaves, wave_g = blockIdx.x * kEvWaves + wave;
    uint4 r0, r1, rec2;
    if constexpr (!FUSED) {
        const uint32_t cap_tiles = (p.dispatch_capacity + kTileRecords - 1) / kTileRecords;
        r0 = setup_load_rec(p, wave_g, wave_g < cap_tiles, p.dispatch_capacity, lane);
        r1 = setup_load_rec(p, wave_g + stride, wave_g + stride < cap_tiles, p.dispatch_capacity, lane);
        rec2 = setup_load_rec(p, wave_g + 2u * stride, wave_g + 2u * stride < cap_tiles, p.dispatch_capacity, lane);
    }
    planes_to_lds(p, planes);
    clear_chunk_sums(p);
    if (threadIdx.x < kEvWaves) s_red[threadIdx.x] = 0u;
    if (CLS && threadIdx.x < 6) cls_sel[threadIdx.x] = ((alpha_bits(p.ci, threadIdx.x >> 1) >> (threadIdx.x & 1u)) & 1u) ? ~0u : 0u;
    const AlphaLds *alpha = alpha_table_fill(p, alpha_tab) ? &alpha_tab : nullptr;
    __syncthreads();
    if constexpr (FUSED) {
        const FusedCullParams &f = *fp;
        const FusedEntity E{p.ci, f.entity_draw_buffer, f.mesh_infos, f.mesh_side, p.entities, f.visibility, f.e_pyr};
        EntityChunksArgs a;
        a.dispatch_buffer = const_cast<uint8_t *>(p.dispatch_buffer);
        a.dispatch_capacity = f.e_dispatch_capacity;
        a.draw_first = f.draw_first, a.draw_limit = f.draw_limit;
        a.ne_chunks = f.ne_chunks;
        a.rec_shift = 5u;
        a.sync = f.sync, a.ent_flags = f.ent_flags, a.total = f.e_total, a.status = p.status;
        const __amdgpu_buffer_rsrc_t DN = rsrc_of(f.done_flags, kShardDoneWords * kShardDoneStride * 4u);
        auto tell_all = [&](uint32_t total) {
            typedef unsigned int v2u __attribute__((ext_vector_type(2)));
            const v2u v = {total, 1u << 8};
            for (uint32_t k = 0; k < kShardDoneWords; k++)
                __builtin_amdgcn_raw_buffer_store_b64(v, DN, k * kShardDoneStride * 4u, 0, kSc1);
        };
        if (blockIdx.x < f.ne_chunks) entity_chunks(E, a, ent_lds, tell_all);
#ifdef ORBIT_TRIAGE
        wall_chunks = wall_clock64();
#endif
        const uint32_t my_copy = (blockIdx.x % kShardDoneWords) * kShardDoneStride * 4u;
        for (uint32_t round = 0;; round++) {
            if (threadIdx.x == 0) {
                if (round == 0u && blockIdx.x >= f.ne_chunks) asm volatile("s_sleep 64" ::: "memory");
                auto w = __builtin_amdgcn_raw_buffer_load_b64(DN, my_copy, 0, kSc1);
                for (uint32_t spins = 0; arrived_chunks(w) == 0u && spins < kShardPatience; spins++) {
                    asm volatile("s_sleep 8" ::: "memory");
                    w = __builtin_amdgcn_raw_buffer_load_b64(DN, my_copy, 0, kSc1);
                }
                s_word[0] = arrived_chunks(w) != 0u ? 1u : 0u;
                s_word[1] = arrived_records(w);
            }
            __syncthreads();
            const uint32_t done = uniform(s_word[0]);
            nrec_raw = uniform(s_word[1]);
            __syncthreads();
            if (done != 0u) break;
            if (round == kSpinLimit / kShardPatience) {
                if (threadIdx.x == 0) latch_status(p.status, ORBIT_E_TIMEOUT);
                nrec_raw = 0u;
                break;
            }
            entity_chunks(E, a, ent_lds, tell_all);
        }
        nrec_raw = min(nrec_raw, f.e_dispatch_capacity);
    }
    const uint32_t nrec = min(nrec_raw, p.dispatch_capacity);
    const uint32_t ntiles = (nrec + kTileRecords - 1) / kTileRecords;
// ... 215 lines not shown
    }
    __builtin_amdgcn_fence(__ATOMIC_RELEASE, "wavefront");
    __builtin_amdgcn_wave_barrier();
    __builtin_amdgcn_fence(__ATOMIC_ACQUIRE, "wavefront");
    return n;
}

__device__ __forceinline__ Pass1Item pass1_load(const MeshletCullParams &p, const WaveTileLds &L,
                                                const uint16_t *list, uint32_t n, uint32_t chunk, int lane) {
    Pass1Item it;
    const uint32_t j = chunk * 64u + (uint32_t)lane;
    const bool valid = j < n;
    it.code = valid ? (uint32_t)list[j] : ~0u;
    const uint32_t rid = (it.code >> 5) & 15u, ml = it.code & 31u;
    const uint4 *src = valid ? reinterpret_cast<const uint4 *>(p.meshlets + (L.r[rid].rec.y + ml))
                             : reinterpret_cast<const uint4 *>(p.zero_page);
    it.a = src[0];
    it.b = src[1];
    return it;
}

template <int PROJ>
__device__ __forceinline__ uint32_t pass1_eval(const MeshletCullParams &p, WaveTileLds &L, const PlaneLds &P,
                                               const AlphaLds *A, int lane, const Pass1Item &it, uint32_t total,
                                               Payload *payload) {
    const bool valid = it.code != ~0u;
    const uint32_t rid = (it.code >> 5) & 15u, ml = it.code & 31u;
    const uint32_t mi = it.b.w & 0xFFFFu;
    const uint32_t abits = A ? (uint32_t)A->bits[mi & (kAlphaTable - 1u)] : alpha_bits(p.ci, p.materials[mi].alpha_mode);
    bool should_draw = false;
    if (valid) {
        Sphere s;
        const bool visible = eval_geometry<1, PROJ>(p, L, P, rid, it.a, it.b, true, s);
        should_draw = should_draw_of(visible, abits, true, false);
    }
    if (should_draw) atomicOr(reinterpret_cast<uint32_t *>(L.draw_mask) + rid, 1u << ml);
    const uint64_t dm = __ballot(should_draw);
    if (payload && should_draw) {
        const uint32_t rank = total + lane_prefix(dm);
        if (rank < kPayloadCap) payload[rank] = make_payload(ml, rid, it.b);
    }
    return total + (uint32_t)__popcll(dm);
}

template <int PROJ, bool LIST = false>
__device__ __forceinline__ void meshlet_pass1_body(const MeshletCullParams &p) {
    __shared__ WaveTileLds lds[kEvWaves][3];
    __shared__ PlaneLds planes;
    __shared__ AlphaLds alpha_tab;
    __shared__ uint16_t s_list[kEvWaves][2][kTileRows * 64];
    __shared__ uint32_t s_red[kEvWaves];
    const int lane = threadIdx.x & 63, wave = threadIdx.x >> 6;
    planes_to_lds(p, planes);
    clear_chunk_sums(p);
    if (threadIdx.x < kEvWaves) s_red[threadIdx.x] = 0u;
    const AlphaLds *alpha = alpha_table_fill(p, alpha_tab) ? &alpha_tab : nullptr;
    __syncthreads();
    const uint32_t nrec = min(*reinterpret_cast<const uint32_t *>(p.dispatch_buffer), p.dispatch_capacity);
    const uint32_t ntiles = (nrec + kTileRecords - 1) / kTileRecords;
    const uint32_t stride = gridDim.x * kEvWaves;
    uint32_t w0 = blockIdx.x * kEvWaves + wave, w1 = w0 + stride, w2 = w1 + stride;
    uint16_t *list_cur = s_list[wave][0], *list_next = s_list[wave][1];
    uint4 rec2;
    uint32_t n_cur;
    Pass1Item cur;
    {
        const uint4 r0 = setup_load_rec(p, w0, w0 < ntiles, nrec, lane);
        const uint4 r1 = setup_load_rec(p, w1, w1 < ntiles, nrec, lane);
        rec2 = setup_load_rec(p, w2, w2 < ntiles, nrec, lane);
        const float4 m0 = setup_load_mat(p, r0, lane);
        const uint32_t p0 = pass1_load_prev(p, r0, lane);
        const float4 m1 = setup_load_mat(p, r1, lane);
        const uint32_t p1 = pass1_load_prev(p, r1, lane);
        setup_write(p, lds[wave][0], r0, m0, lane, p0);
        setup_write(p, lds[wave][1], r1, m1, lane, p1);
        n_cur = pass1_build_list(lds[wave][0], list_cur, lane);
        cur = pass1_load(p, lds[wave][0], list_cur, n_cur, 0u, lane);
    }
    uint32_t it = 0;
    while (w0 < ntiles) {
        const uint32_t w3 = w2 + stride;
        WaveTileLds &L = lds[wave][it % 3];
        WaveTileLds &Ln = lds[wave][(it + 1) % 3];
        Payload *payload = p.task_records ? nullptr : p.tile_payload + (size_t)w0 * kPayloadCap;
        const float4 mat2 = setup_load_mat(p, rec2, lane);
        const uint32_t prev2 = pass1_load_prev(p, rec2, lane);
        const uint4 rec3 = setup_load_rec(p, w3, w3 < ntiles, nrec, lane);
        uint32_t total = 0, n_next = 0;
        for (uint32_t chunk = 0;; chunk++) {
            const bool last = (chunk + 1u) * 64u >= n_cur;
            Pass1Item next;
            if (!last) {
                next = pass1_load(p, L, list_cur, n_cur, chunk + 1u, lane);
            } else {
                n_next = pass1_build_list(Ln, list_next, lane);
                next = pass1_load(p, Ln, list_next, n_next, 0u, lane);
            }
            total = pass1_eval<PROJ>(p, L, planes, alpha, lane, cur, total, payload);
            cur = next;
            if (last) break;
        }
        setup_write(p, lds[wave][(it + 2) % 3], rec2, mat2, lane, prev2);
        if ((p.task_records != nullptr || total > kPayloadCap) && lane < 2 * (int)kTileRows)
            p.tile_masks[(size_t)w0 * (2 * kTileRows) + lane] = reinterpret_cast<const uint32_t *>(L.draw_mask)[lane];
        if (lane == 0) p.tile_counts[w0] = total;
        if (LIST && p.visible_list == 2u) tile_records_out(p, L, nrec, w0, total, s_red + wave, lane);
        uint16_t *t = list_cur;
// ... 21 lines not shown

uint32_t eval_grid(uint32_t pass, bool stream, uint32_t max_tiles, uint32_t num_cus) {
    uint32_t wps = (uint32_t)ev_waves_per_simd((int)pass, stream);
    if (wps > (uint32_t)kEvWavesPerSimd && max_tiles < 8u * num_cus * wps * (uint32_t)kEvWaves) wps = (uint32_t)kEvWavesPerSimd;
    uint32_t blocks = num_cus * wps;
    const uint32_t need = (max_tiles + kEvWaves - 1) / kEvWaves;
    if (blocks > need) blocks = need;
    return blocks == 0 ? 1u : blocks;
}

template <int PASS>
void launch_eval_pass(const MeshletCullParams &p, dim3 grid, hipStream_t s) {
    const dim3 block(kEvWaves * 64);
    const bool ortho = p.ci.projection_type == 1;
    if constexpr (PASS == 1) {
        if (ortho)
            hipLaunchKernelGGL((meshlet_pass1_kernel<1>), grid, block, 0, s, p);
        else
            hipLaunchKernelGGL((meshlet_pass1_kernel<0>), grid, block, 0, s, p);
    } else if (p.ms.sphere != nullptr && p.ms.cls0 != nullptr) {
        if (ortho)
            hipLaunchKernelGGL((meshlet_eval_kernel<PASS, 1, false, true, true>), grid, block, 0, s, p);
        else
            hipLaunchKernelGGL((meshlet_eval_kernel<PASS, 0, false, true, true>), grid, block, 0, s, p);
    } else if (p.ms.sphere != nullptr) {
        if (ortho)
            hipLaunchKernelGGL((meshlet_eval_kernel<PASS, 1, false, true>), grid, block, 0, s, p);
        else
            hipLaunchKernelGGL((meshlet_eval_kernel<PASS, 0, false, true>), grid, block, 0, s, p);
    } else if constexpr (PASS == 0) {
#ifdef ORBIT_TRIAGE
        if (p.debug_flags & 8u) {
            if (ortho)
                hipLaunchKernelGGL((meshlet_eval_kernel<0, 1, true>), grid, block, 0, s, p);
            else
                hipLaunchKernelGGL((meshlet_eval_kernel<0, 0, true>), grid, block, 0, s, p);
        } else
#endif
        if (ortho) {
            hipLaunchKernelGGL((meshlet_eval_kernel<0, 1, false>), grid, block, 0, s, p);
        } else {
            hipLaunchKernelGGL((meshlet_eval_kernel<0, 0, false>), grid, block, 0, s, p);
        }
    } else {
        if (ortho)
            hipLaunchKernelGGL((meshlet_eval_kernel<PASS, 1, false>), grid, block, 0, s, p);
        else
            hipLaunchKernelGGL((meshlet_eval_kernel<PASS, 0, false>), grid, block, 0, s, p);
    }
}

}

hipError_t launch_meshlet_eval(const MeshletCullParams &p, uint32_t num_cus, hipStream_t s) {
#if !ORBIT_CONTRACT
    if (p.arith != 0u) return launch_meshlet_eval_contracted(p, num_cus, s);
#endif
    const uint32_t max_tiles = (p.dispatch_capacity + kTileRecords - 1) / kTileRecords;
    const uint32_t pass = p.ci.occlusion_pass;
    const dim3 grid(eval_grid(pass, p.ms.sphere != nullptr, max_tiles, num_cus));
#ifndef ORBIT_PASS2_BY_VALUE
    if (p.visible_list == 2u) {
        MeshletCullViews one{};
        one.v[0] = p;
        const ViewGroup g{};
        const int src = p.ms.sphere == nullptr ? 0 : (p.ms.cls0 != nullptr ? 2 : 1);
        return launch_meshlet_eval_views(one, g, 1u, pass, p.ci.projection_type == 1, src, max_tiles, num_cus, s);
    }
    if (pass == 2u) {
        MeshletCullViews one{};
        one.v[0] = p;
        ViewGroup g{};
        const int src = p.ms.sphere == nullptr ? 0 : (p.ms.cls0 != nullptr ? 2 : 1);
        const dim3 block(kEvWaves * 64);
        const bool ortho = p.ci.projection_type == 1;
        if (src == 2) {
            if (ortho) hipLaunchKernelGGL((meshlet_eval_views_kernel<2, 1, true, true>), grid, block, 0, s, one, g);
            else hipLaunchKernelGGL((meshlet_eval_views_kernel<2, 0, true, true>), grid, block, 0, s, one, g);
        } else if (src == 1) {
            if (ortho) hipLaunchKernelGGL((meshlet_eval_views_kernel<2, 1, true>), grid, block, 0, s, one, g);
            else hipLaunchKernelGGL((meshlet_eval_views_kernel<2, 0, true>), grid, block, 0, s, one, g);
        } else {
            if (ortho) hipLaunchKernelGGL((meshlet_eval_views_kernel<2, 1, false>), grid, block, 0, s, one, g);
            else hipLaunchKernelGGL((meshlet_eval_views_kernel<2, 0, false>), grid, block, 0, s, one, g);
        }
        return hipGetLastError();
    }
#endif
    switch (pass) {
    case 0: launch_eval_pass<0>(p, grid, s); break;
    case 1: launch_eval_pass<1>(p, grid, s); break;
    default: launch_eval_pass<2>(p, grid, s); break;
    }
    return hipGetLastError();
}

hipError_t launch_shard_cull(const FusedCullParams &f, uint32_t num_cus, hipStream_t s) {
#if !ORBIT_CONTRACT
    if (f.m.arith != 0u) return launch_shard_cull_contracted(f, num_cus, s);
#endif
    const MeshletCullParams &p = f.m;
    const uint32_t max_tiles = (p.dispatch_capacity + kTileRecords - 1) / kTileRecords;
    const dim3 grid(max(eval_grid(0u, p.ms.sphere != nullptr, max_tiles, num_cus), min(f.ne_chunks, num_cus * (uint32_t)kEvWavesPerSimd))), block(kEvWaves * 64);
    ShardCullArgs a{};
    a.v[0] = f;
    const ViewGroup g{};
// ... 50 lines not shown
```

### orbit_amd/csrc/meshlet_stream.hip

```cpp
#include "kernels.h"

namespace orbit {

namespace {

struct StreamBuildArrays {
    uint4 *sphere;
    uint32_t *cone;
    uint16_t *mat;
    uint32_t *cmd;
    uint16_t *cnt;
    uint32_t *link, *cls0, *cls1;
    uint2 *base32;
    uint64_t s_first, s_end;
    const OrbitMaterialData *materials;
    uint32_t material_count;
    uint32_t *other;
};

__device__ __forceinline__ uint32_t alpha_class(const StreamBuildArrays &A, uint32_t material_index) {
    if (A.materials == nullptr || material_index >= A.material_count) return 3u;
    const uint32_t mode = A.materials[material_index].alpha_mode;
    return mode < 3u ? mode : 3u;
}

__global__ __launch_bounds__(256) void meshlet_stream_build_kernel(const OrbitMeshlet *meshlets, uint64_t first,
                                                                   uint64_t count, const StreamBuildArrays A) {
    const int lane = threadIdx.x & 63;
    const uint64_t lo = first & ~63ull, end = first + count;
    for (uint64_t base = lo + ((uint64_t)blockIdx.x * 256u + (threadIdx.x & ~63u)); base <= end;
         base += (uint64_t)gridDim.x * 256u) {
        const uint64_t m = base + (uint64_t)lane;
        const bool in = m >= first && m < end;
        uint32_t vtx = 0, data = 0, cls = 3u;
        if (in) {
            const uint4 *src = reinterpret_cast<const uint4 *>(meshlets + m);
            const uint4 a = src[0], b = src[1];
            A.sphere[m] = a;
            A.cone[m] = b.x;
            A.mat[m] = (uint16_t)(b.w & 0xFFFFu);
            A.cmd[m * 3u] = b.y;
            A.cmd[m * 3u + 1u] = b.z;
            A.cmd[m * 3u + 2u] = b.w;
            A.cnt[m] = (uint16_t)(b.w >> 16);
            if ((m & 31u) == 0u) A.base32[m >> 5] = make_uint2(b.y, b.z);
            vtx = b.y, data = b.z;
            cls = alpha_class(A, b.w & 0xFFFFu);
            if (cls == 3u && A.materials != nullptr) *A.other = 1u;
        } else if (m == end && m < A.s_end) {
            vtx = A.cmd[m * 3u], data = A.cmd[m * 3u + 1u];
        }
        const bool in_stream = m >= A.s_first && m < A.s_end;
// ... 27 lines not shown
            A.link[(base >> 5) + 1u] = (uint32_t)(mask >> 32);
            A.cls0[(base >> 5) + 1u] = (uint32_t)(m0 >> 32);
            A.cls1[(base >> 5) + 1u] = (uint32_t)(m1 >> 32);
        }
    }
}

__global__ __launch_bounds__(256) void meshlet_stream_classes_kernel(const StreamBuildArrays A) {
    const int lane = threadIdx.x & 63;
    for (uint64_t base = (A.s_first & ~63ull) + ((uint64_t)blockIdx.x * 256u + (threadIdx.x & ~63u)); base < A.s_end;
         base += (uint64_t)gridDim.x * 256u) {
        const uint64_t m = base + (uint64_t)lane;
        const bool in = m >= A.s_first && m < A.s_end;
        const uint32_t cls = in ? alpha_class(A, (uint32_t)A.mat[m]) : 3u;
        if (in && cls == 3u && A.materials != nullptr) *A.other = 1u;
        const uint64_t m0 = __ballot((cls & 1u) != 0u), m1 = __ballot((cls & 2u) != 0u);
        if (lane == 0 && base + 32u > A.s_first) {
            A.cls0[base >> 5] = (uint32_t)m0;
            A.cls1[base >> 5] = (uint32_t)m1;
        }
        if (lane == 32 && base + 32u < A.s_end) {
            A.cls0[(base >> 5) + 1u] = (uint32_t)(m0 >> 32);
            A.cls1[(base >> 5) + 1u] = (uint32_t)(m1 >> 32);
        }
    }
}

}

static StreamBuildArrays stream_build_arrays(const MeshletStreamView &ms, const OrbitMaterialData *materials,
                                             uint32_t material_count, uint32_t *other = nullptr) {
    return StreamBuildArrays{const_cast<uint4 *>(ms.sphere),   const_cast<uint32_t *>(ms.cone),
                             const_cast<uint16_t *>(ms.mat),   const_cast<uint32_t *>(ms.cmd),
                             const_cast<uint16_t *>(ms.cnt),   const_cast<uint32_t *>(ms.link),
                             const_cast<uint32_t *>(ms.cls0),  const_cast<uint32_t *>(ms.cls1),
                             const_cast<uint2 *>(ms.base32),
                             (uint64_t)ms.first,               (uint64_t)ms.first + ms.count,
                             materials,                        material_count,
                             other};
}

hipError_t launch_meshlet_stream_build(const OrbitMeshlet *meshlets, uint64_t first, uint64_t count,
                                       const MeshletStreamView &ms, const OrbitMaterialData *materials,
                                       uint32_t material_count, uint32_t *other, hipStream_t s) {
    if (count == 0) return hipSuccess;
    const uint64_t need = (count + 64u + 255u) / 256u + 1u;
    const uint32_t blocks = (uint32_t)(need < 8192u ? need : 8192u);
    hipLaunchKernelGGL(meshlet_stream_build_kernel, dim3(blocks), dim3(256), 0, s, meshlets, first, count,
                       stream_build_arrays(ms, materials, material_count, other));
    return hipGetLastError();
}

__global__ __launch_bounds__(256) void meshlet_stream_validate_kernel(const OrbitMeshlet *meshlets, const StreamBuildArrays A,
                                                                      int32_t *status) {
    for (uint64_t m = A.s_first + (uint64_t)blockIdx.x * 256u + threadIdx.x; m < A.s_end; m += (uint64_t)gridDim.x * 256u) {
        const uint4 *src = reinterpret_cast<const uint4 *>(meshlets + m);
        const uint4 a = src[0], b = src[1], sa = A.sphere[m];
        bool same = a.x == sa.x && a.y == sa.y && a.z == sa.z && a.w == sa.w && b.x == A.cone[m] &&
                    (b.w & 0xFFFFu) == (uint32_t)A.mat[m] && b.y == A.cmd[m * 3u] && b.z == A.cmd[m * 3u + 1u] &&
                    b.w == A.cmd[m * 3u + 2u] && (b.w >> 16) == (uint32_t)A.cnt[m];
        if (A.materials) {
            const uint32_t cls = ((A.cls0[m >> 5] >> (m & 31u)) & 1u) | (((A.cls1[m >> 5] >> (m & 31u)) & 1u) << 1);
            same = same && cls == alpha_class(A, b.w & 0xFFFFu);
        }
        if ((m & 31u) == 0u) {
            const uint2 b32 = A.base32[m >> 5];
            same = same && b32.x == b.y && b32.y == b.z;
        }
        if (m > A.s_first) {
            const uint4 pb = reinterpret_cast<const uint4 *>(meshlets + (m - 1u))[1];
            const bool link = b.y == pb.y && b.z == pb.z + meshlet_data_words((pb.w >> 16) & 0xFFu, pb.w >> 24);
            same = same && link == (((A.link[m >> 5] >> (m & 31u)) & 1u) != 0u);
        }
        if (!same) latch_status(status, ORBIT_E_STALE);
    }
}

hipError_t launch_meshlet_stream_validate(const OrbitMeshlet *meshlets, const MeshletStreamView &ms,
                                          const OrbitMaterialData *materials, uint32_t material_count, int32_t *status,
                                          hipStream_t s) {
    if (ms.count == 0) return hipSuccess;
    const uint64_t need = ((uint64_t)ms.count + 255u) / 256u;
    const uint32_t blocks = (uint32_t)(need < 8192u ? need : 8192u);
    hipLaunchKernelGGL(meshlet_stream_validate_kernel, dim3(blocks), dim3(256), 0, s, meshlets,
                       stream_build_arrays(ms, materials, material_count), status);
    return hipGetLastError();
}

hipError_t launch_meshlet_stream_classes(const MeshletStreamView &ms, const OrbitMaterialData *materials,
                                         uint32_t material_count, uint32_t *other, hipStream_t s) {
    const uint64_t need = ((uint64_t)ms.count + 64u + 255u) / 256u + 1u;
    const uint32_t blocks = (uint32_t)(need < 8192u ? need : 8192u);
    hipLaunchKernelGGL(meshlet_stream_classes_kernel, dim3(blocks), dim3(256), 0, s,
                       stream_build_arrays(ms, materials, material_count, other));
    return hipGetLastError();
}

namespace {

__global__ __launch_bounds__(256) void mesh_side_build_kernel(const OrbitMeshInfo *mesh_infos, uint32_t first, uint32_t count,
                                                             MeshSide *table) {
    const uint32_t i = blockIdx.x * 256u + threadIdx.x;
    if (i >= count) return;
    const OrbitMeshInfo &m = mesh_infos[first + i];
    MeshSide s;
    s.sphere[0] = m.bounding_sphere[0], s.sphere[1] = m.bounding_sphere[1], s.sphere[2] = m.bounding_sphere[2], s.sphere[3] = m.bounding_sphere[3];
    s.lod_count = m.lod_count;
    s.lod0_offset = m.mesh_lods[0].meshlet_offset;
    s.lod0_count = m.mesh_lods[0].meshlet_count;
    s.valid = 1u;
    table[first + i] = s;
}

__global__ __launch_bounds__(256) void mesh_side_validate_kernel(const OrbitMeshInfo *mesh_infos, uint32_t first, uint32_t count,
                                                                const MeshSide *table, int32_t *status) {
    const uint32_t i = blockIdx.x * 256u + threadIdx.x;
    if (i >= count) return;
    const OrbitMeshInfo &m = mesh_infos[first + i];
    const MeshSide s = table[first + i];
    if (s.valid == 0u) return;
    bool same = s.lod_count == m.lod_count && s.lod0_offset == m.mesh_lods[0].meshlet_offset && s.lod0_count == m.mesh_lods[0].meshlet_count;
    for (int k = 0; k < 4; k++) same = same && __float_as_uint(s.sphere[k]) == __float_as_uint(m.bounding_sphere[k]);
    if (!same) latch_status(status, ORBIT_E_STALE);
}

}

hipError_t launch_mesh_side_build(const OrbitMeshInfo *mesh_infos, uint32_t first, uint32_t count, MeshSide *table, hipStream_t s) {
    if (count == 0) return hipSuccess;
    hipLaunchKernelGGL(mesh_side_build_kernel, dim3((count + 255u) / 256u), dim3(256), 0, s, mesh_infos, first, count, table);
    return hipGetLastError();
}

hipError_t launch_mesh_side_validate(const OrbitMeshInfo *mesh_infos, uint32_t first, uint32_t count, const MeshSide *table,
                                     int32_t *status, hipStream_t s) {
    if (count == 0) return hipSuccess;
    hipLaunchKernelGGL(mesh_side_validate_kernel, dim3((count + 255u) / 256u), dim3(256), 0, s, mesh_infos, first, count, table, status);
    return hipGetLastError();
// ... 4 lines not shown
```

### orbit_amd/engine.py

```python
import ctypes as C

import numpy as np

from . import _lib, layouts


def _ptr(t):
    if t is None:
        return None
    if isinstance(t, int):
        return C.c_void_p(t)
    return C.c_void_p(t.data_ptr())


def _stream(stream):
    import torch

    s = torch.cuda.current_stream() if stream is None else stream
    return C.c_void_p(s.cuda_stream)


def _host_bytes(x, nbytes):
    a = np.ascontiguousarray(x).view(np.uint8).reshape(-1)
    if a.nbytes != nbytes:
# ... 472 lines not shown
                           record_capacity, draw_commands_buffer=None, draw_capacity=0, material_count=0,
                           visibility_buffer=None, meshlet_visibility_buffer=None, depth_pyramid=None,
                           depth_pyramid_size=(0, 0), stream=None):
        if stream is None:
            raise ValueError("prepare_cull_shard: pass the stream the prepared call enqueues on")
        return PreparedShardCull(self, cull_info, entity_draw_buffer, mesh_info_buffer, meshlet_dispatch_buffer, entity_buffer,
                                 draw_first, draw_count, dispatch_capacity, meshlet_buffer, material_buffer, record_buffer,
                                 record_capacity, draw_commands_buffer, draw_capacity, material_count, visibility_buffer,
                                 meshlet_visibility_buffer, depth_pyramid, depth_pyramid_size, stream)

    def mesh_side_culls(self):
        return int(self._lib.orbit_ctx_mesh_side_culls(self._ctx))

    def shard_culls(self):
        return int(self._lib.orbit_ctx_shard_culls(self._ctx))

    def expand_visible_records(self, record_buffer, meshlet_buffer, draw_commands_buffer, draw_capacity, stream=None):
        _lib.check(self._lib.orbit_expand_visible_records(self._ctx, _ptr(record_buffer), _ptr(meshlet_buffer),
                                                          _ptr(draw_commands_buffer), draw_capacity, _stream(stream)),
                   self._ctx)

    def p2p_alloc(self, nbytes):
        ptr, handle = C.c_void_p(), (C.c_uint8 * 64)()
        _lib.check(self._lib.orbit_p2p_alloc(self._ctx, int(nbytes), C.byref(ptr), handle), self._ctx)
        return int(ptr.value), bytes(handle)

    def p2p_free(self, ptr):
        _lib.check(self._lib.orbit_p2p_free(self._ctx, C.c_void_p(ptr)), self._ctx)

    def p2p_open(self, handle):
        ptr, h = C.c_void_p(), (C.c_uint8 * 64).from_buffer_copy(handle)
        _lib.check(self._lib.orbit_p2p_open(self._ctx, h, C.byref(ptr)), self._ctx)
        return int(ptr.value)

    def p2p_close(self, ptr):
        _lib.check(self._lib.orbit_p2p_close(self._ctx, C.c_void_p(ptr)), self._ctx)

    def meshlet_stream(self, meshlet_buffer, first, count, stream=None):
        return MeshletStream(self, meshlet_buffer, first, count, stream)

    def bind_meshlet_stream(self, ms):
        _lib.check(self._lib.orbit_ctx_bind_meshlet_stream(self._ctx, ms._h if ms is not None else None), self._ctx)
        self._meshlet_stream = ms

    def fused_culls(self):
        return int(self._lib.orbit_ctx_fused_culls(self._ctx))

    def meshlet_stream_culls(self):
        return int(self._lib.orbit_ctx_meshlet_stream_culls(self._ctx))

    def meshlet_class_culls(self):
        return int(self._lib.orbit_ctx_meshlet_class_culls(self._ctx))

    def exchange_list(self, local_list, rank, world, out_buffers, ctrl_buffers, out_capacity, header_bytes, stride,
                      stream=None):
        outs = (C.c_void_p * world)(*[_ptr(b) for b in out_buffers])
        ctrls = (C.c_void_p * world)(*[_ptr(b) for b in ctrl_buffers])
        _lib.check(self._lib.orbit_exchange_list(self._ctx, _ptr(local_list), rank, world, outs, ctrls, out_capacity,
                                                 header_bytes, stride, _stream(stream)), self._ctx)

    def prepare_exchange_list(self, local_list, rank, world, out_buffers, ctrl_buffers, out_capacity, header_bytes, stride,
                              stream=None):
        outs = (C.c_void_p * world)(*[_ptr(b) for b in out_buffers])
        ctrls = (C.c_void_p * world)(*[_ptr(b) for b in ctrl_buffers])
        fn, ctx, lst, st = self._lib.orbit_exchange_list, self._ctx, _ptr(local_list), _stream(stream)
        keep = (outs, ctrls, local_list, stream)

        def call():
            rc = fn(ctx, lst, rank, world, outs, ctrls, out_capacity, header_bytes, stride, st)
            if rc != _lib.OK:
                _lib.check(rc, ctx)
            return keep

        return call

    def allgather_list(self, nccl_comm, rank, world, local_list, segment_capacity, segments, out_list, out_capacity,
                       header_bytes, stride, stream=None):
        comm = nccl_comm if isinstance(nccl_comm, C.c_void_p) else C.c_void_p(int(nccl_comm))
        _lib.check(self._lib.orbit_allgather_list(self._ctx, comm, rank, world, _ptr(local_list), segment_capacity,
                                                  _ptr(segments), _ptr(out_list), out_capacity, header_bytes, stride,
                                                  _stream(stream)), self._ctx)

    def compact_segments(self, segments, world, segment_capacity, out_list, out_capacity, header_bytes, stride,
                         stream=None):
        _lib.check(self._lib.orbit_compact_segments(self._ctx, _ptr(segments), world, segment_capacity, _ptr(out_list),
                                                    out_capacity, header_bytes, stride, _stream(stream)), self._ctx)

    def gather_visible(self, nccl_comm, rank, world, local_draw_buffer, out_draw_buffer, out_capacity, stream=None):
        comm = nccl_comm if isinstance(nccl_comm, C.c_void_p) else C.c_void_p(int(nccl_comm))
        _lib.check(self._lib.orbit_gather_visible(self._ctx, comm, rank, world, _ptr(local_draw_buffer),
                                                  _ptr(out_draw_buffer), out_capacity, _stream(stream)), self._ctx)

    def compute_clusters(self, push, info, depth, lights, tile_depth_slice_mask, depth_bounds, unique_cluster_buffer,
                         index_capacity, light_index_buffer, light_index_capacity, cluster_offset_image, stream=None):
        pc = _host_bytes(push, layouts.MARK_ACTIVE_PUSH.itemsize)
        ib = _host_bytes(info, layouts.CLUSTER_CULL_INFO.itemsize)
        _lib.check(self._lib.orbit_compute_clusters(
            self._ctx, pc.ctypes.data_as(C.c_void_p), ib.ctypes.data_as(C.c_void_p), _ptr(depth), _ptr(lights),
            _ptr(tile_depth_slice_mask), _ptr(depth_bounds), _ptr(unique_cluster_buffer), index_capacity,
            _ptr(light_index_buffer), light_index_capacity, _ptr(cluster_offset_image), _stream(stream)), self._ctx)

    def cluster_stats(self, stats, push, info, depth, lights, stream=None):
        if stats.numel() * stats.element_size() < layouts.CLUSTER_STATS.itemsize:
            raise ValueError("stats needs 256 bytes")
        pc = _host_bytes(push, layouts.MARK_ACTIVE_PUSH.itemsize)
        ib = _host_bytes(info, layouts.CLUSTER_CULL_INFO.itemsize)
# ... 24 lines not shown
```

### orbit_amd/host/orbit_host_c.cpp

```cpp
#include "orbit_host_c.h"

#include <cstring>
#include <map>
#include <memory>
#include <string>

#include "orbit_host.hpp"
#include "orbit_assets.hpp"
#include "orbit_gltf.hpp"
#include "orbit_raster.hpp"
#include "orbit_scene.hpp"

using namespace orbit;
using namespace orbit::passes;

namespace {
thread_local std::string g_err = "no error";

struct HostCtx {
    std::unique_ptr<graphics::Context> ctx;
    std::map<std::string, std::unique_ptr<DepthPyramid>> pyramids;
};

camera::Projection to_projection(const OrbitHostProjection &p) {
    return p.kind == 0 ? camera::Projection::perspective(p.fov, p.near_clip)
                       : camera::Projection::orthographic(p.half_width, p.near_clip, p.far_clip);
}

CullInfo to_cull_info(const OrbitHostCullInfo &h) {
    CullInfo ci;
    ci.view_matrix = Mat4::from_cols_array(h.view_matrix);
    for (uint32_t i = 0; i < h.plane_count && i < 16; i++)
        ci.view_space_cull_planes.push_back({h.view_space_cull_planes[i][0], h.view_space_cull_planes[i][1],
                                             h.view_space_cull_planes[i][2], h.view_space_cull_planes[i][3]});
    ci.projection = to_projection(h.projection);
    ci.occlusion_culling.kind = (OcclusionCullInfo::Kind)h.occlusion_kind;
    ci.occlusion_culling.visibility_buffer.ptr = h.visibility_buffer;
    ci.occlusion_culling.meshlet_visibility_buffer.ptr = h.meshlet_visibility_buffer;
    ci.occlusion_culling.depth_pyramid.ptr = h.depth_pyramid;
    ci.occlusion_culling.depth_pyramid.width = h.depth_pyramid_size[0];
    ci.occlusion_culling.depth_pyramid.height = h.depth_pyramid_size[1];
    ci.occlusion_culling.noskip_alphamode.bits = h.noskip_alphamode;
    ci.occlusion_culling.aspect_ratio = h.aspect_ratio;
    ci.alpha_mode_filter.bits = h.alpha_mode_filter;
    ci.lod_range_start = h.lod_range[0];
    ci.lod_range_end = h.lod_range[1];
    ci.lod_base = h.lod_base;
    ci.lod_step = h.lod_step;
    ci.lod_target_pos_view_space = {h.lod_target_pos_view_space[0], h.lod_target_pos_view_space[1],
                                    h.lod_target_pos_view_space[2]};
    return ci;
}
AssetGraphData to_assets(const OrbitHostAssets &a) {
    AssetGraphData o;
    o.meshlet_buffer.ptr = a.meshlet_buffer;
    o.mesh_info_buffer.ptr = a.mesh_info_buffer;
    o.materials_buffer.ptr = a.materials_buffer;
    o.material_count = a.material_count;
    return o;
}
SceneGraphData to_scene(const OrbitHostScene &s) {
    SceneGraphData o;
    o.entity_draw_count = s.entity_draw_count;
    o.entity_draw_buffer.ptr = s.entity_draw_buffer;
// ... 545 lines not shown
    out->materials = s.assets.materials.size();
    out->vertices = s.assets.vertex_positions.size() / 3;
    out->entities = s.entities.size();
}
const OrbitMeshInfo *orbit_host_gltf_mesh_infos(const void *scene) {
    return static_cast<const gltf_loader::LoadedScene *>(scene)->assets.mesh_infos.data();
}
const OrbitMeshlet *orbit_host_gltf_meshlets(const void *scene) {
    return static_cast<const gltf_loader::LoadedScene *>(scene)->assets.meshlets.data();
}
const uint32_t *orbit_host_gltf_meshlet_data(const void *scene) {
    return static_cast<const gltf_loader::LoadedScene *>(scene)->assets.meshlet_data.data();
}
const OrbitMaterialData *orbit_host_gltf_materials(const void *scene) {
    return static_cast<const gltf_loader::LoadedScene *>(scene)->assets.materials.data();
}
const float *orbit_host_gltf_vertex_positions(const void *scene) {
    return static_cast<const gltf_loader::LoadedScene *>(scene)->assets.vertex_positions.data();
}
uint64_t orbit_host_gltf_entities(const void *scene, OrbitHostGltfEntity *out, uint64_t capacity) {
    const auto &s = *static_cast<const gltf_loader::LoadedScene *>(scene);
    for (size_t i = 0; i < s.entities.size() && i < capacity; i++) {
        const auto &e = s.entities[i];
        out[i].mesh = e.mesh;
        const float p[3] = {e.transform.position.x, e.transform.position.y, e.transform.position.z};
        const float q[4] = {e.transform.orientation.x, e.transform.orientation.y, e.transform.orientation.z,
                            e.transform.orientation.w};
        const float sc[3] = {e.transform.scale.x, e.transform.scale.y, e.transform.scale.z};
        std::memcpy(out[i].position, p, 12);
        std::memcpy(out[i].orientation, q, 16);
        std::memcpy(out[i].scale, sc, 12);
    }
    return s.entities.size();
}
uint64_t orbit_host_simplify_clustered(const float *positions, uint64_t vertex_count, const uint32_t *indices,
                                       uint64_t index_count, uint64_t target_index_count, uint32_t *out,
                                       uint64_t capacity, uint64_t *needed) {
    std::vector<uint32_t> r;
    assets::simplify_clustered(positions, (size_t)vertex_count, indices, (size_t)index_count,
                               (size_t)target_index_count, r);
    if (needed) *needed = r.size();
    const size_t n = std::min<size_t>(r.size(), (size_t)capacity) / 3 * 3;
    if (out && n) std::memcpy(out, r.data(), n * 4);
    return n;
}
void orbit_host_transform_from_mat4(const float matrix[16], float position[3], float orientation[4], float scale[3]) {
    const passes::Transform t = gltf_loader::transform_from_mat4(Mat4::from_cols_array(matrix));
    position[0] = t.position.x, position[1] = t.position.y, position[2] = t.position.z;
    orientation[0] = t.orientation.x, orientation[1] = t.orientation.y, orientation[2] = t.orientation.z;
    orientation[3] = t.orientation.w;
    scale[0] = t.scale.x, scale[1] = t.scale.y, scale[2] = t.scale.z;
}

}
```

### orbit_amd/host/orbit_host_c.h

```cpp
#ifndef ORBIT_HOST_C_H
#define ORBIT_HOST_C_H
#include "../../include/orbit_abi_ext.h"
#ifdef __cplusplus
extern "C" {
#endif

#define ORBIT_HOST_PANIC (-100)

typedef struct OrbitHostProjection {
    uint32_t kind;
    float fov, half_width, near_clip, far_clip;
} OrbitHostProjection;

typedef struct OrbitHostCullInfo {
    float view_matrix[16];
    float view_space_cull_planes[16][4];
    uint32_t plane_count;
    OrbitHostProjection projection;
    uint32_t occlusion_kind;
    void *visibility_buffer;
    void *meshlet_visibility_buffer;
    float *depth_pyramid;
    uint32_t depth_pyramid_size[2];
    uint32_t noskip_alphamode;
// ... 135 lines not shown
const OrbitSceneEntity *orbit_host_scene_entity_table(const void *scene, uint64_t *count);
uint64_t orbit_host_scene_shadow_orientations(const void *scene, float *orientations, uint64_t capacity);
int64_t orbit_host_scene_light_index(const void *scene, uint64_t entity);

int32_t orbit_host_compute_meshlets(const float *positions, uint64_t vertex_count, const uint32_t *indices,
                                    uint64_t index_count, uint32_t material, uint32_t vertex_offset,
                                    uint32_t data_offset_base, OrbitMeshlet *out_meshlets, uint32_t *out_meshlet_data,
                                    uint64_t *meshlet_count, uint64_t *meshlet_data_words);
void orbit_host_compute_mesh_bounds(const float *positions, uint64_t vertex_count, float aabb_min[3], float aabb_max[3],
                                    float bounding_sphere[4]);

int32_t orbit_host_meshlet_bounds(const OrbitMeshlet *meshlets, uint64_t meshlet_capacity, const uint32_t *indices,
                                  uint64_t first, uint64_t count, const uint32_t *meshlet_data, uint64_t meshlet_data_words,
                                  const void *vertices, uint64_t vertex_count, uint32_t vertex_stride,
                                  uint32_t position_offset, OrbitMeshletBoundsFull *out, int32_t *range_error,
                                  uint32_t *updates);

int32_t orbit_host_raster_depth(const void *draw_commands, uint32_t max_commands, const uint32_t *meshlet_data,
                                uint64_t meshlet_data_words, const void *vertices, uint64_t vertex_count,
                                uint32_t vertex_stride, uint32_t position_offset, const OrbitEntityData *entity_data,
                                uint32_t entity_count, const float view_proj[16], float *depth, uint32_t width,
                                uint32_t height, uint32_t flags, OrbitRasterStats *stats, int32_t *command_error);

int32_t orbit_host_raster_visibility(const void *draw_commands, uint32_t max_commands, const uint32_t *meshlet_data,
                                     uint64_t meshlet_data_words, const void *vertices, uint64_t vertex_count,
                                     uint32_t vertex_stride, uint32_t position_offset, const OrbitEntityData *entity_data,
                                     uint32_t entity_count, const float view_proj[16], uint64_t *visibility, uint32_t width,
                                     uint32_t height, uint32_t flags, uint32_t command_base, OrbitRasterStats *stats,
                                     int32_t *command_error);
int32_t orbit_host_visibility_resolve(const uint64_t *visibility, uint32_t width, uint32_t height, uint32_t command_base,
                                      uint32_t max_commands, float *depth, uint32_t *command_pixels,
                                      OrbitVisibilityStats *stats);

typedef struct OrbitHostGltfCounts {
    uint64_t meshes, meshlets, meshlet_data_words, materials, vertices, entities;
} OrbitHostGltfCounts;
typedef struct OrbitHostGltfEntity {
    int32_t mesh;
    float position[3], orientation[4], scale[3];
} OrbitHostGltfEntity;
void *orbit_host_gltf_load(const char *path);
void orbit_host_gltf_free(void *scene);
void orbit_host_gltf_counts(const void *scene, OrbitHostGltfCounts *out);
const OrbitMeshInfo *orbit_host_gltf_mesh_infos(const void *scene);
const OrbitMeshlet *orbit_host_gltf_meshlets(const void *scene);
const uint32_t *orbit_host_gltf_meshlet_data(const void *scene);
const OrbitMaterialData *orbit_host_gltf_materials(const void *scene);
const float *orbit_host_gltf_vertex_positions(const void *scene);
uint64_t orbit_host_gltf_entities(const void *scene, OrbitHostGltfEntity *out, uint64_t capacity);
uint64_t orbit_host_simplify_clustered(const float *positions, uint64_t vertex_count, const uint32_t *indices,
                                       uint64_t index_count, uint64_t target_index_count, uint32_t *out,
                                       uint64_t capacity, uint64_t *needed);
void orbit_host_transform_from_mat4(const float matrix[16], float position[3], float orientation[4], float scale[3]);
#ifdef __cplusplus
}
#endif
#endif
```

Before: 195.2 billion.

## Add per-32-meshlet block bounds pretest to skip per-meshlet cone/frustum work

Builds a bounding sphere per 32-meshlet block when the meshlet stream is updated. A new block-evaluation kernel uses these bounds to decide frustum-inside and sparse cone tests once per block instead of per meshlet. It is enabled by default for non-occlusion perspective command culls and can be turned off with ORBIT_BLOCK_CULL=0. The cost is extra memory per meshlet, a build kernel at every stream update and more conservative-bound arithmetic. Scenes with loose blocks gain little and may take some overhead.

```diff
diff --git a/bindings/rust/orbit_hip.rs b/bindings/rust/orbit_hip.rs
--- a/bindings/rust/orbit_hip.rs
+++ b/bindings/rust/orbit_hip.rs
@@ -238,6 +238,10 @@
     pub fn orbit_frame_late(ctx: *mut OrbitCtx, frame: *const OrbitFrameLate, stream: *mut c_void) -> i32;
     pub fn orbit_ctx_meshlet_stream_culls(ctx: *const OrbitCtx) -> u64;
     pub fn orbit_ctx_meshlet_class_culls(ctx: *const OrbitCtx) -> u64;
+    pub fn orbit_ctx_block_culls(ctx: *const OrbitCtx) -> u64;
+    pub fn orbit_ctx_set_block_cull(ctx: *mut OrbitCtx, enable: u32) -> i32;
+    pub fn orbit_meshlet_stream_block_bounds(ctx: *mut OrbitCtx, ms: *mut OrbitMeshletStream, first_block: u64, count: u64,
+                                             out: *mut c_void, stream: *mut c_void) -> i32;
     pub fn orbit_p2p_alloc(ctx: *mut OrbitCtx, bytes: u64, out_ptr: *mut *mut c_void, out_handle: *mut [u8; 64]) -> i32;
     pub fn orbit_p2p_free(ctx: *mut OrbitCtx, ptr: *mut c_void) -> i32;
     pub fn orbit_p2p_open(ctx: *mut OrbitCtx, handle: *const [u8; 64], out_peer_ptr: *mut *mut c_void) -> i32;
diff --git a/include/orbit_abi_ext.h b/include/orbit_abi_ext.h
--- a/include/orbit_abi_ext.h
+++ b/include/orbit_abi_ext.h
@@ -46,6 +46,10 @@
 int32_t orbit_ctx_bind_meshlet_stream(OrbitCtx *ctx, OrbitMeshletStream *ms);
 uint64_t orbit_ctx_meshlet_stream_culls(const OrbitCtx *ctx);
 uint64_t orbit_ctx_meshlet_class_culls(const OrbitCtx *ctx);
+uint64_t orbit_ctx_block_culls(const OrbitCtx *ctx);
+int32_t orbit_ctx_set_block_cull(OrbitCtx *ctx, uint32_t enable);
+int32_t orbit_meshlet_stream_block_bounds(OrbitCtx *ctx, OrbitMeshletStream *ms, uint64_t first_block, uint64_t count,
+                                          void *out, void *stream);
 
 typedef struct OrbitDepthReduceItem {
     const float *depth;
diff --git a/orbit_amd/_lib.py b/orbit_amd/_lib.py
--- a/orbit_amd/_lib.py
+++ b/orbit_amd/_lib.py
@@ -180,6 +180,10 @@
     "orbit_ctx_bind_meshlet_stream": (C.c_int32, [C.c_void_p, C.c_void_p]),
     "orbit_ctx_meshlet_stream_culls": (C.c_uint64, [C.c_void_p]),
     "orbit_ctx_meshlet_class_culls": (C.c_uint64, [C.c_void_p]),
+    "orbit_ctx_block_culls": (C.c_uint64, [C.c_void_p]),
+    "orbit_ctx_set_block_cull": (C.c_int32, [C.c_void_p, C.c_uint32]),
+    "orbit_meshlet_stream_block_bounds": (C.c_int32, [C.c_void_p, C.c_void_p, C.c_uint64, C.c_uint64, C.c_void_p,
+                                                      C.c_void_p]),
     "orbit_cull_shard": (C.c_int32, [C.c_void_p, C.c_void_p, C.POINTER(EntityCullBufs), C.c_uint32, C.c_uint32,
                                      C.POINTER(MeshletCullBufs), C.c_void_p, C.c_uint32, C.c_uint32, C.c_void_p]),
     "orbit_ctx_shard_culls": (C.c_uint64, [C.c_void_p]),
diff --git a/orbit_amd/csrc/abi_ctx.hip b/orbit_amd/csrc/abi_ctx.hip
--- a/orbit_amd/csrc/abi_ctx.hip
+++ b/orbit_amd/csrc/abi_ctx.hip
@@ -160,6 +160,8 @@
     const char *dbg = getenv("ORBIT_SP_DEBUG");
     ctx->debug_flags = dbg ? (uint32_t)atoi(dbg) : 0u;
 #endif
+    const char *bc = getenv("ORBIT_BLOCK_CULL");
+    ctx->block_cull = !(bc && bc[0] == '0' && bc[1] == '\0');
     snprintf(ctx->err, sizeof(ctx->err), "no error");
     const OrbitCaps child_caps = view_child_caps(caps);
     for (uint32_t v = 1; v < caps.max_views; v++) {
diff --git a/orbit_amd/csrc/abi_cull.hip b/orbit_amd/csrc/abi_cull.hip
--- a/orbit_amd/csrc/abi_cull.hip
+++ b/orbit_amd/csrc/abi_cull.hip
@@ -207,7 +207,8 @@
 int32_t validate_stream(OrbitCtx *ctx, const MeshletCullParams &p, hipStream_t s) {
     if (!p.ms.sphere || !ctx->caps.validate_streams) return ORBIT_OK;
     const hipError_t e = launch_meshlet_stream_validate(p.meshlets, p.ms, p.ms.cls0 ? p.materials : nullptr,
-                                                        ctx->meshlet_stream->material_count, ctx->status, s);
+                                                        ctx->meshlet_stream->material_count, ctx->status, s,
+                                                        stream_block_bounds(ctx->meshlet_stream));
     return e == hipSuccess ? ORBIT_OK : hip_fail(ctx, e, "launch meshlet_stream_validate");
 }
 
@@ -245,9 +246,12 @@
     hipError_t e = hipSuccess;
     if (ctx->rec_shift > 5u) e = launch_split_records(split_params_for(ctx, ctx, b), s);
     if (e != hipSuccess) return hip_fail(ctx, e, "launch split_records");
-    e = launch_meshlet_cull(p, ctx->num_cus, s, ev0, ev1);
+    const bool blocks = ctx->block_cull && out.kind == MeshletCullOut::kCommands && p.ms.sphere != nullptr &&
+                        p.ms.cls0 != nullptr && ci->occlusion_pass == 0u && ci->projection_type == 0u && p.arith == 0u;
+    e = launch_meshlet_cull(p, ctx->num_cus, s, ev0, ev1, blocks ? stream_block_bounds(ctx->meshlet_stream) : nullptr);
     if (e != hipSuccess) return hip_fail(ctx, e, "launch meshlet_cull");
     count_stream_cull(ctx, p);
+    if (blocks) ctx->block_culls++;
     return ORBIT_OK;
 }
 
diff --git a/orbit_amd/csrc/abi_internal.h b/orbit_amd/csrc/abi_internal.h
--- a/orbit_amd/csrc/abi_internal.h
+++ b/orbit_amd/csrc/abi_internal.h
@@ -8,6 +8,7 @@
 #include <new>
 #include <vector>
 
+#include "block_pretest.h"
 #include "kernels.h"
 
 using namespace orbit;
@@ -24,6 +25,7 @@
     uint16_t *cnt = nullptr;
     uint32_t *link = nullptr, *cls0 = nullptr, *cls1 = nullptr;
     uint2 *base32 = nullptr;
+    BlockBound *blk = nullptr;
     std::mutex mu;
     const void *source = nullptr;
     uint64_t valid_lo = 0, valid_hi = 0;
@@ -88,6 +90,8 @@
     OrbitMeshletStream *meshlet_stream = nullptr;
     uint64_t stream_culls = 0;
     uint64_t class_culls = 0;
+    uint64_t block_culls = 0;
+    bool block_cull = true;
     char err[512] = {0};
 };
 
@@ -151,6 +155,8 @@
     return v;
 }
 
+inline const BlockBound *stream_block_bounds(const OrbitMeshletStream *ms) { return ms->blk - (ms->first >> 5); }
+
 struct PreparedCullViews {
     EntityCullViews ev{};
     MeshletCullViews mv{};
diff --git a/orbit_amd/csrc/abi_stream.hip b/orbit_amd/csrc/abi_stream.hip
--- a/orbit_amd/csrc/abi_stream.hip
+++ b/orbit_amd/csrc/abi_stream.hip
@@ -54,6 +54,7 @@
                   {(void **)&ms->cnt, capacity * sizeof(uint16_t) + 256u, 0},
                   {(void **)&ms->link, bit_words * sizeof(uint32_t), 0},
                   {(void **)&ms->base32, bit_words * sizeof(uint2), 0},
+                  {(void **)&ms->blk, bit_words * sizeof(BlockBound), 0},
                   {(void **)&ms->cls0, bit_words * sizeof(uint32_t), 0xFF},
                   {(void **)&ms->cls1, bit_words * sizeof(uint32_t), 0xFF}};
     for (auto &a : arrays) {
@@ -67,7 +68,7 @@
     if (e == hipSuccess) e = hipEventCreateWithFlags(&ms->other_event, hipEventDisableTiming);
     if (e != hipSuccess) {
         orbit_meshlet_stream_destroy(ms);
-        return hip_fail(ctx, e, "meshlet_stream_create: hipMalloc (36.65 B per meshlet)");
+        return hip_fail(ctx, e, "meshlet_stream_create: hipMalloc (37.65 B per meshlet)");
     }
     *out_stream = ms;
     return ORBIT_OK;
@@ -93,6 +94,13 @@
                                                (const OrbitMaterialData *)ms->materials, ms->material_count, ms->d_other,
                                                (hipStream_t)stream);
     if (e != hipSuccess) return hip_fail(ctx, e, "launch meshlet_stream_build");
+    if (count != 0) {
+        const MeshletStreamView all = stream_arrays(ms, ms->first, ms->first + ms->capacity);
+        e = launch_block_bounds_build(all.sphere, const_cast<BlockBound *>(stream_block_bounds(ms)), first >> 5,
+                                      ((first + count - 1u) >> 5) - (first >> 5) + 1u, ms->first, ms->first + ms->capacity,
+                                      (hipStream_t)stream);
+        if (e != hipSuccess) return hip_fail(ctx, e, "launch block_bounds_build");
+    }
     if (ms->materials != nullptr && count != 0) {
         e = read_back_class_flag(ms, (hipStream_t)stream);
         if (e != hipSuccess) return hip_fail(ctx, e, "meshlet_stream_update: class flag read-back");
@@ -208,8 +216,24 @@
     }
     const hipError_t e = launch_meshlet_stream_validate((const OrbitMeshlet *)meshlet_buffer, v,
                                                         classes ? (const OrbitMaterialData *)material_buffer : nullptr,
-                                                        ms->material_count, ctx->status, (hipStream_t)stream);
+                                                        ms->material_count, ctx->status, (hipStream_t)stream,
+                                                        stream_block_bounds(ms));
     if (e != hipSuccess) return hip_fail(ctx, e, "launch meshlet_stream_validate");
+    return ORBIT_OK;
+}
+
+int32_t orbit_meshlet_stream_block_bounds(OrbitCtx *ctx, OrbitMeshletStream *ms, uint64_t first_block, uint64_t count,
+                                          void *out, void *stream) {
+    if (!ctx) return fail(nullptr, ORBIT_E_INVALID, "ctx is NULL");
+    std::lock_guard<std::mutex> lock(ctx->mu);
+    if (const int32_t rc = check_stream(ctx, ms, "meshlet_stream_block_bounds", true, out)) return rc;
+    const uint64_t b0 = ms->first >> 5, b1 = (ms->first + ms->capacity + 31u) >> 5;
+    if (first_block < b0 || count > b1 - b0 || first_block - b0 > b1 - b0 - count)
+        return fail(ctx, ORBIT_E_CAPACITY, "meshlet_stream_block_bounds: blocks [%llu, +%llu) outside the stream's [%llu, %llu)",
+                    (unsigned long long)first_block, (unsigned long long)count, (unsigned long long)b0, (unsigned long long)b1);
+    hipError_t e = hipStreamSynchronize((hipStream_t)stream);
+    if (e == hipSuccess) e = hipMemcpy(out, ms->blk + (first_block - b0), count * sizeof(BlockBound), hipMemcpyDeviceToHost);
+    if (e != hipSuccess) return hip_fail(ctx, e, "meshlet_stream_block_bounds: read-back");
     return ORBIT_OK;
 }
 
@@ -225,6 +249,7 @@
     (void)hipFree(ms->cnt);
     (void)hipFree(ms->link);
     (void)hipFree(ms->base32);
+    (void)hipFree(ms->blk);
     (void)hipFree(ms->cls0);
     (void)hipFree(ms->cls1);
     (void)hipFree(ms->d_other);
@@ -249,5 +274,13 @@
 uint64_t orbit_ctx_meshlet_stream_culls(const OrbitCtx *ctx) { return ctx ? ctx->stream_culls : 0; }
 uint64_t orbit_ctx_meshlet_class_culls(const OrbitCtx *ctx) { return ctx ? ctx->class_culls : 0; }
 uint64_t orbit_ctx_shard_culls(const OrbitCtx *ctx) { return ctx ? ctx->shard_culls : 0; }
-
-}
+uint64_t orbit_ctx_block_culls(const OrbitCtx *ctx) { return ctx ? ctx->block_culls : 0; }
+
+int32_t orbit_ctx_set_block_cull(OrbitCtx *ctx, uint32_t enable) {
+    if (!ctx) return fail(nullptr, ORBIT_E_INVALID, "ctx is NULL");
+    std::lock_guard<std::mutex> lock(ctx->mu);
+    ctx->block_cull = enable != 0u;
+    return ORBIT_OK;
+}
+
+}
diff --git a/orbit_amd/csrc/block_pretest.h b/orbit_amd/csrc/block_pretest.h
--- /dev/null
+++ b/orbit_amd/csrc/block_pretest.h
@@ -0,0 +1,161 @@
+#pragma once
+#include <math.h>
+#include <stdint.h>
+#include <string.h>
+
+#if defined(__HIPCC__) || defined(__CUDACC__)
+#define ORBIT_BLK_FN __host__ __device__ inline
+#else
+#define ORBIT_BLK_FN inline
+#endif
+
+namespace orbit {
+
+ORBIT_BLK_FN uint32_t blk_bits(float f) {
+    uint32_t u;
+    __builtin_memcpy(&u, &f, 4);
+    return u;
+}
+ORBIT_BLK_FN float blk_float(uint32_t u) {
+    float f;
+    __builtin_memcpy(&f, &u, 4);
+    return f;
+}
+ORBIT_BLK_FN uint32_t blk_up16(float x) { return (blk_bits(x) + 0xFFFFu) >> 16; }
+
+struct BlockBound {
+    float cx, cy, cz;
+    uint32_t packed;
+    float rc;
+    float r_max;
+    uint32_t valid;
+    uint32_t pad_;
+};
+static_assert(sizeof(BlockBound) == 32, "BlockBound layout");
+
+ORBIT_BLK_FN BlockBound block_bound_unpack(float cx, float cy, float cz, uint32_t packed) {
+    BlockBound b;
+    b.cx = cx, b.cy = cy, b.cz = cz, b.packed = packed;
+    b.rc = blk_float(packed & 0xFFFF0000u);
+    b.r_max = blk_float(packed << 16);
+    b.valid = (packed >> 16) != 0u ? 1u : 0u;
+    b.pad_ = 0u;
+    return b;
+}
+
+struct BlockRecord {
+    float gx, gy, gz, dk;
+    float sigma;
+    float bk;
+    float rr;
+    uint32_t flags;
+};
+static_assert(sizeof(BlockRecord) == 32, "BlockRecord layout");
+constexpr uint32_t kBlkSparse = 1u;
+constexpr uint32_t kBlkInside = 2u;
+
+constexpr float kBlkEps = 0x1p-18f;
+constexpr float kBlkSlack = 1.0f + 0x1p-10f;
+constexpr float kBlkUp = 1.0f + 0x1p-20f;
+constexpr float kBlkTiny = 0x1p-80f;
+constexpr float kBlkHuge = 0x1p60f;
+#ifndef ORBIT_BLK_RATIO
+#define ORBIT_BLK_RATIO 8.0f
+#endif
+
+ORBIT_BLK_FN float blk_max(float a, float b) { return a > b ? a : b; }
+
+ORBIT_BLK_FN BlockBound block_bound_finish(float cx, float cy, float cz, float dist_max, float r_max, float r_min, bool finite) {
+    BlockBound b;
+    b.cx = cx, b.cy = cy, b.cz = cz;
+    b.rc = dist_max * kBlkUp + 0x1p-60f;
+    b.r_max = r_max;
+    const bool ok = finite && r_min >= 0.0f && b.rc < kBlkHuge && r_max < kBlkHuge && fabsf(cx) < kBlkHuge &&
+                    fabsf(cy) < kBlkHuge && fabsf(cz) < kBlkHuge;
+    b.valid = ok ? 1u : 0u;
+    b.packed = ok ? (blk_up16(b.rc) << 16 | blk_up16(r_max)) : 0u;
+    b.pad_ = 0u;
+    return b;
+}
+ORBIT_BLK_FN float block_dist(float cx, float cy, float cz, float x, float y, float z) {
+    const float dx = x - cx, dy = y - cy, dz = z - cz;
+    return sqrtf(fmaf(dz, dz, fmaf(dy, dy, dx * dx)));
+}
+
+ORBIT_BLK_FN BlockBound block_bound_of(const float *spheres, uint32_t n) {
+    const float inf = INFINITY;
+    float lo[3] = {inf, inf, inf}, hi[3] = {-inf, -inf, -inf}, r_max = 0.0f, r_min = 0.0f;
+    bool finite = true;
+    for (uint32_t i = 0; i < n; i++) {
+        const float *s = spheres + 4 * i;
+        for (int k = 0; k < 3; k++) lo[k] = fminf(lo[k], s[k]), hi[k] = fmaxf(hi[k], s[k]);
+        r_max = fmaxf(r_max, s[3]), r_min = fminf(r_min, s[3]);
+        finite = finite && isfinite(s[0]) && isfinite(s[1]) && isfinite(s[2]) && isfinite(s[3]);
+    }
+    const float cx = 0.5f * lo[0] + 0.5f * hi[0], cy = 0.5f * lo[1] + 0.5f * hi[1], cz = 0.5f * lo[2] + 0.5f * hi[2];
+    float dist = 0.0f;
+    for (uint32_t i = 0; i < n; i++) dist = fmaxf(dist, block_dist(cx, cy, cz, spheres[4 * i], spheres[4 * i + 1], spheres[4 * i + 2]));
+    return block_bound_finish(cx, cy, cz, dist, r_max, r_min, finite);
+}
+
+ORBIT_BLK_FN BlockRecord block_record_setup(const float *m, bool affine, float scale, const BlockBound &b, bool covered,
+                                            const float *planes, uint32_t n_planes, float ratio = ORBIT_BLK_RATIO) {
+    BlockRecord o;
+    const float Cx = b.cx, Cy = b.cy, Cz = b.cz;
+    const float dx = fmaf(m[8], Cz, fmaf(m[4], Cy, fmaf(m[0], Cx, m[12])));
+    const float dy = fmaf(m[9], Cz, fmaf(m[5], Cy, fmaf(m[1], Cx, m[13])));
+    const float dz = fmaf(m[10], Cz, fmaf(m[6], Cy, fmaf(m[2], Cx, m[14])));
+    const float aCx = fabsf(Cx), aCy = fabsf(Cy), aCz = fabsf(Cz);
+    const float apx = fmaf(fabsf(m[8]), aCz, fmaf(fabsf(m[4]), aCy, fmaf(fabsf(m[0]), aCx, fabsf(m[12]))));
+    const float apy = fmaf(fabsf(m[9]), aCz, fmaf(fabsf(m[5]), aCy, fmaf(fabsf(m[1]), aCx, fabsf(m[13]))));
+    const float apz = fmaf(fabsf(m[10]), aCz, fmaf(fabsf(m[6]), aCy, fmaf(fabsf(m[2]), aCx, fabsf(m[14]))));
+    const float g00 = fmaf(m[2], m[2], fmaf(m[1], m[1], m[0] * m[0]));
+    const float g11 = fmaf(m[6], m[6], fmaf(m[5], m[5], m[4] * m[4]));
+    const float g22 = fmaf(m[10], m[10], fmaf(m[9], m[9], m[8] * m[8]));
+    const float g01 = fabsf(fmaf(m[2], m[6], fmaf(m[1], m[5], m[0] * m[4])));
+    const float g02 = fabsf(fmaf(m[2], m[10], fmaf(m[1], m[9], m[0] * m[8])));
+    const float g12 = fabsf(fmaf(m[6], m[10], fmaf(m[5], m[9], m[4] * m[8])));
+    const float s2 = blk_max(g00 + g01 + g02, blk_max(g11 + g01 + g12, g22 + g02 + g12));
+    const float sigma = sqrtf(s2) * (1.0f + 0x1p-16f) + 0x1p-60f;
+    const float ap = (blk_max(apx, blk_max(apy, apz)) + 2.0f * sigma * b.rc) * kBlkUp;
+    const float rcp = fmaf(kBlkEps, ap, sigma * b.rc * kBlkUp);
+    const float D = sqrtf(fmaf(dz, dz, fmaf(dy, dy, dx * dx)));
+    const float gx = fmaf(m[2], dz, fmaf(m[1], dy, m[0] * dx));
+    const float gy = fmaf(m[6], dz, fmaf(m[5], dy, m[4] * dx));
+    const float gz = fmaf(m[10], dz, fmaf(m[9], dy, m[8] * dx));
+    const float kf = 0x1.020408p-7f;
+    const float mag = ap + D + rcp;
+    o.gx = gx * kf, o.gy = gy * kf, o.gz = gz * kf, o.dk = D * kf;
+    o.sigma = sigma;
+    o.bk = kf * fmaf(kBlkEps, mag, rcp) * kBlkSlack;
+    o.rr = b.r_max * scale * kBlkSlack + kBlkTiny;
+    bool sparse = affine && covered && b.valid != 0u && D > ratio * rcp && D > 0x1p-40f && mag < kBlkHuge &&
+                  sigma < 0x1p40f && o.rr < kBlkHuge && scale >= 0.0f;
+    bool inside = sparse;
+    for (uint32_t i = 0; i < n_planes; i++) {
+        const float nx = planes[4 * i], ny = planes[4 * i + 1], nz = planes[4 * i + 2], w = planes[4 * i + 3];
+        const float nn = sqrtf(fmaf(nz, nz, fmaf(ny, ny, nx * nx))) * kBlkUp + kBlkTiny;
+        const float dist = fmaf(nz, dz, fmaf(ny, dy, fmaf(nx, dx, w))) - nn * rcp;
+        const float margin = fmaf(kBlkEps, fmaf(nn, mag, fabsf(w)), kBlkTiny);
+        inside = inside && dist > margin;
+    }
+    o.flags = (sparse ? kBlkSparse : 0u) | (inside ? kBlkInside : 0u);
+    return o;
+}
+
+ORBIT_BLK_FN void block_pretest_terms(const BlockRecord &r, uint32_t cone, float &s0, float &band) {
+    const float ax = (float)(int)(int8_t)(cone & 0xFFu), ay = (float)(int)(int8_t)((cone >> 8) & 0xFFu);
+    const float az = (float)(int)(int8_t)((cone >> 16) & 0xFFu), co = (float)(int)(int8_t)(cone >> 24);
+    s0 = fmaf(r.gx, ax, fmaf(r.gy, ay, fmaf(r.gz, az, -(co * r.dk))));
+    const float a1 = fabsf(ax) + fabsf(ay) + fabsf(az);
+    band = fmaf(r.bk, fmaf(r.sigma, a1, fabsf(co)), kBlkTiny);
+}
+ORBIT_BLK_FN bool block_cone_culls(const BlockRecord &r, float s0, float band) { return s0 >= band + r.rr; }
+ORBIT_BLK_FN bool block_cone_keeps(float s0, float band) { return s0 < -band; }
+ORBIT_BLK_FN uint32_t block_pretest(const BlockRecord &r, uint32_t cone) {
+    float s0, band;
+    block_pretest_terms(r, cone, s0, band);
+    return block_cone_culls(r, s0, band) ? 1u : (block_cone_keeps(s0, band) ? 2u : 0u);
+}
+
+}
diff --git a/orbit_amd/csrc/kernels.h b/orbit_amd/csrc/kernels.h
--- a/orbit_amd/csrc/kernels.h
+++ b/orbit_amd/csrc/kernels.h
@@ -7,6 +7,8 @@
 #include "orbit_device.h"
 
 namespace orbit {
+
+struct BlockBound;
 
 constexpr uint32_t kTileRecords = 16;
 constexpr uint32_t kTileRows = 8;
@@ -234,7 +236,7 @@
 hipError_t launch_entity_cull_views(const EntityCullViews &all, uint32_t n, uint32_t max_entity_draw_count,
                                     uint32_t num_cus, hipStream_t s);
 hipError_t launch_meshlet_cull(const MeshletCullParams &p, uint32_t num_cus, hipStream_t s,
-                               hipEvent_t ev0 = nullptr, hipEvent_t ev1 = nullptr);
+                               hipEvent_t ev0 = nullptr, hipEvent_t ev1 = nullptr, const BlockBound *blk = nullptr);
 struct MeshletCullViews {
     MeshletCullParams v[ORBIT_MAX_CULL_VIEWS];
 };
@@ -243,6 +245,8 @@
     uint8_t idx[ORBIT_MAX_CULL_VIEWS];
 };
 hipError_t launch_meshlet_eval(const MeshletCullParams &p, uint32_t num_cus, hipStream_t s);
+hipError_t launch_meshlet_eval_blocks(const MeshletCullParams &p, const BlockBound *blk, dim3 grid, hipStream_t s);
+uint32_t meshlet_eval_blocks_grid(uint32_t max_tiles, uint32_t num_cus);
 hipError_t launch_meshlet_eval_views(const MeshletCullViews &all, const ViewGroup &g, uint32_t m, uint32_t pass,
                                      bool ortho, int src, uint32_t max_tiles, uint32_t num_cus, hipStream_t s);
 hipError_t launch_meshlet_emit(const MeshletCullParams &p, bool stream, uint32_t num_cus, hipStream_t s);
@@ -255,7 +259,9 @@
                                        uint32_t material_count, uint32_t *other, hipStream_t s);
 hipError_t launch_meshlet_stream_validate(const OrbitMeshlet *meshlets, const MeshletStreamView &ms,
                                           const OrbitMaterialData *materials, uint32_t material_count, int32_t *status,
-                                          hipStream_t s);
+                                          hipStream_t s, const BlockBound *blk = nullptr);
+hipError_t launch_block_bounds_build(const uint4 *sphere, BlockBound *blk, uint64_t block_first, uint64_t block_count,
+                                     uint64_t s_first, uint64_t s_end, hipStream_t s);
 hipError_t launch_scene_update_entities(const OrbitEntityTransform *transforms, const uint32_t *instance_indices,
                                         uint32_t count, OrbitEntityData *entity_data, uint32_t entity_capacity,
                                         int32_t *status, hipStream_t s);
diff --git a/orbit_amd/csrc/meshlet_common.h b/orbit_amd/csrc/meshlet_common.h
--- a/orbit_amd/csrc/meshlet_common.h
+++ b/orbit_amd/csrc/meshlet_common.h
@@ -420,6 +420,14 @@
         if (p.task_records && rec.z < 32u) word |= ~0u << rec.z;
         if (rec.z > 0) p.meshlet_visibility[rec.w] = word;
     }
+}
+
+__device__ __forceinline__ void clear_chunk_sums(const MeshletCullParams &p, uint32_t threads) {
+    if (blockIdx.x != 0) return;
+    const uint32_t max_tiles = (p.dispatch_capacity + kTileRecords - 1) / kTileRecords;
+    const uint32_t max_chunks = (max_tiles + kScanChunk - 1) / kScanChunk;
+    for (uint32_t c = threadIdx.x; c < max_chunks; c += threads) p.chunk_sums[c] = 0u;
+    if (threadIdx.x < kEmitTicketPools) p.tickets[(kTicketPools + threadIdx.x) * kTicketStride] = 0u;
 }
 
 __device__ __forceinline__ uint4 setup_load_rec(const MeshletCullParams &p, uint32_t tile, bool tile_valid,
diff --git a/orbit_amd/csrc/meshlet_cull.hip b/orbit_amd/csrc/meshlet_cull.hip
--- a/orbit_amd/csrc/meshlet_cull.hip
+++ b/orbit_amd/csrc/meshlet_cull.hip
@@ -28,12 +28,20 @@
 }
 
 hipError_t launch_meshlet_cull(const MeshletCullParams &p, uint32_t num_cus, hipStream_t s, hipEvent_t ev0,
-                               hipEvent_t ev1) {
+                               hipEvent_t ev1, const BlockBound *blk) {
     const uint32_t max_tiles = (p.dispatch_capacity + kTileRecords - 1) / kTileRecords;
     if ((max_tiles + kScanChunk - 1) / kScanChunk > kEmitChunkTable) return hipErrorInvalidValue;
     hipError_t e;
     if (ev0 && (e = hipEventRecord(ev0, s)) != hipSuccess) return e;
-    if ((e = launch_meshlet_eval(p, num_cus, s)) != hipSuccess) return e;
+    if (blk != nullptr) {
+        if (p.ci.occlusion_pass != 0u || p.ci.projection_type != 0u || p.arith != 0u || p.ms.cls0 == nullptr ||
+            p.visible_list != 0u || p.task_records != nullptr)
+            return hipErrorInvalidValue;
+        e = launch_meshlet_eval_blocks(p, blk, dim3(meshlet_eval_blocks_grid(max_tiles, num_cus)), s);
+    } else {
+        e = launch_meshlet_eval(p, num_cus, s);
+    }
+    if (e != hipSuccess) return e;
     if (ev1 && (e = hipEventRecord(ev1, s)) != hipSuccess) return e;
     if (p.task_records) return launch_task_records(p, s);
     if (p.visible_list == 2u) {
diff --git a/orbit_amd/csrc/meshlet_eval.hip b/orbit_amd/csrc/meshlet_eval.hip
--- a/orbit_amd/csrc/meshlet_eval.hip
+++ b/orbit_amd/csrc/meshlet_eval.hip
@@ -12,14 +12,6 @@
 #endif
 constexpr int ev_waves_per_simd(int pass, bool stream) { return (pass == 0 && stream) ? ORBIT_EV_WPS0 : kEvWavesPerSimd; }
 
-
-__device__ __forceinline__ void clear_chunk_sums(const MeshletCullParams &p) {
-    if (blockIdx.x != 0) return;
-    const uint32_t max_tiles = (p.dispatch_capacity + kTileRecords - 1) / kTileRecords;
-    const uint32_t max_chunks = (max_tiles + kScanChunk - 1) / kScanChunk;
-    for (uint32_t c = threadIdx.x; c < max_chunks; c += kEvWaves * 64) p.chunk_sums[c] = 0u;
-    if (threadIdx.x < kEmitTicketPools) p.tickets[(kTicketPools + threadIdx.x) * kTicketStride] = 0u;
-}
 
 constexpr uint32_t kShardPatience = 256;
 
@@ -63,7 +55,7 @@
         rec2 = setup_load_rec(p, wave_g + 2u * stride, wave_g + 2u * stride < cap_tiles, p.dispatch_capacity, lane);
     }
     planes_to_lds(p, planes);
-    clear_chunk_sums(p);
+    clear_chunk_sums(p, kEvWaves * 64);
     if (threadIdx.x < kEvWaves) s_red[threadIdx.x] = 0u;
     if (CLS && threadIdx.x < 6) cls_sel[threadIdx.x] = ((alpha_bits(p.ci, threadIdx.x >> 1) >> (threadIdx.x & 1u)) & 1u) ? ~0u : 0u;
     const AlphaLds *alpha = alpha_table_fill(p, alpha_tab) ? &alpha_tab : nullptr;
@@ -385,7 +377,7 @@
     __shared__ uint32_t s_red[kEvWaves];
     const int lane = threadIdx.x & 63, wave = threadIdx.x >> 6;
     planes_to_lds(p, planes);
-    clear_chunk_sums(p);
+    clear_chunk_sums(p, kEvWaves * 64);
     if (threadIdx.x < kEvWaves) s_red[threadIdx.x] = 0u;
     const AlphaLds *alpha = alpha_table_fill(p, alpha_tab) ? &alpha_tab : nullptr;
     __syncthreads();
@@ -513,6 +505,10 @@
 
 }
 
+#if !ORBIT_CONTRACT
+uint32_t meshlet_eval_blocks_grid(uint32_t max_tiles, uint32_t num_cus) { return eval_grid(0u, true, max_tiles, num_cus); }
+#endif
+
 hipError_t launch_meshlet_eval(const MeshletCullParams &p, uint32_t num_cus, hipStream_t s) {
 #if !ORBIT_CONTRACT
     if (p.arith != 0u) return launch_meshlet_eval_contracted(p, num_cus, s);
diff --git a/orbit_amd/csrc/meshlet_eval_blocks.hip b/orbit_amd/csrc/meshlet_eval_blocks.hip
--- /dev/null
+++ b/orbit_amd/csrc/meshlet_eval_blocks.hip
@@ -0,0 +1,278 @@
+#include "block_pretest.h"
+#include "meshlet_common.h"
+
+namespace orbit {
+
+namespace {
+
+constexpr int kBkWaves = 4;
+constexpr int kBkWavesPerSimd = 5;
+constexpr uint32_t kBkRing = 512, kBkFlush = 64;
+
+struct __attribute__((aligned(16))) BlockTileLds {
+    BlockRecord r[kTileRecords];
+};
+struct CandRing {
+    uint16_t code[kBkRing];
+};
+struct RingState {
+    uint32_t head = 0, count = 0;
+    uint32_t total = 0;
+};
+
+__device__ __forceinline__ bool row_is_sparse(const WaveTileLds &L, int r) {
+    const uint32_t w = reinterpret_cast<const uint32_t *>(&L.pad_)[0];
+    return (((uint32_t)__builtin_amdgcn_readfirstlane((int)w) >> (2 * r)) & 1u) != 0u;
+}
+
+struct BoundRegs {
+    float4 q;
+};
+__device__ __forceinline__ BoundRegs blk_load_bound(const MeshletCullParams &p, const BlockBound *blk, const uint4 &rec, int lane) {
+    const int src_lane = (lane & 15) * 4;
+    const uint32_t y = (uint32_t)__shfl((int)rec.y, src_lane, 64), z = (uint32_t)__shfl((int)rec.z, src_lane, 64);
+    const uint32_t rel = y - p.ms.first;
+    BoundRegs b;
+    const bool covered = lane < (int)kTileRecords && z != 0u && (y & 31u) == 0u && rel < p.ms.count && z <= p.ms.count - rel;
+    const float4 *src = covered ? reinterpret_cast<const float4 *>(blk + (y >> 5)) : reinterpret_cast<const float4 *>(p.zero_page);
+    b.q = src[0];
+    return b;
+}
+
+__device__ __forceinline__ void blk_setup(const MeshletCullParams &p, WaveTileLds &L, BlockTileLds &B, const PlaneLds &P,
+                                          const BoundRegs &bb, int lane) {
+    uint32_t flags = 0u;
+    if (lane < (int)kTileRecords) {
+        const RecordLds &R = L.r[lane];
+        float m[16];
+#pragma unroll
+        for (int c = 0; c < 4; c++) {
+            const float4 col = R.mcol[c];
+            m[4 * c] = col.x, m[4 * c + 1] = col.y, m[4 * c + 2] = col.z, m[4 * c + 3] = col.w;
+        }
+        const BlockBound b = block_bound_unpack(bb.q.x, bb.q.y, bb.q.z, __float_as_uint(bb.q.w));
+        const uint32_t aw = reinterpret_cast<const uint32_t *>(&L.affine_rows)[lane >> 3];
+        const bool affine = ((aw >> (8 * ((lane >> 1) & 3))) & 1u) != 0u;
+        BlockRecord o = block_record_setup(m, affine, R.scale, b, true, reinterpret_cast<const float *>(P.plane),
+                                           min(p.ci.cull_plane_count, (uint32_t)ORBIT_MAX_CULL_PLANES));
+        if (R.rec.z == 0u) o.flags = kBlkSparse;
+        B.r[lane] = o;
+        flags = o.flags;
+    }
+    uint64_t m = __ballot((flags & kBlkSparse) != 0u);
+    m &= m >> 1;
+    if (lane == 0) L.pad_ = m & 0x5555ull;
+    __builtin_amdgcn_fence(__ATOMIC_RELEASE, "wavefront");
+    __builtin_amdgcn_wave_barrier();
+    __builtin_amdgcn_fence(__ATOMIC_ACQUIRE, "wavefront");
+}
+
+template <int R>
+__device__ __forceinline__ void blk_row_load(const MeshletCullParams &p, const WaveTileLds &L, bool sparse, int lane,
+                                             RowRegs<1> &t, const StreamRsrc &SR) {
+    const uint32_t half = lane >> 5, ml = lane & 31;
+    const uint4 rec = L.r[2 * R + half].rec;
+    const bool active = ml < rec.z;
+    const uint32_t rel = rec.y + ml - SR.first;
+    const bool in = active & (rel < SR.count);
+    if (active & !in) latch_status(p.status, ORBIT_E_RANGE);
+    const uint32_t i = in ? rel : kNoOffset >> 4;
+    const uint32_t is = sparse ? kNoOffset >> 4 : i;
+    const auto sp = __builtin_amdgcn_raw_buffer_load_b128(SR.sphere, is << 4, 0, ORBIT_EVAL_LOAD_AUX);
+    const uint32_t c = __builtin_amdgcn_raw_buffer_load_b32(SR.cone, i << 2, 0, ORBIT_EVAL_LOAD_AUX);
+    t.a[0] = make_uint4(sp[0], sp[1], sp[2], sp[3]);
+    t.b[0] = make_uint4(c, 0u, 0u, 0u);
+    t.prev[0] = 0u;
+}
+
+template <int R>
+__device__ __forceinline__ void blk_row_eval(WaveTileLds &L, const BlockTileLds &B, CandRing &ring, int lane,
+                                             const RowRegs<1> &t, RingState &rs) {
+    const uint32_t half = lane >> 5;
+    const BlockRecord br = B.r[2 * R + half];
+    float s0, band;
+    block_pretest_terms(br, t.b[0].x, s0, band);
+    const uint64_t culled = ballot(block_cone_culls(br, s0, band));
+    const uint64_t kept = ballot(block_cone_keeps(s0, band)) & ballot((br.flags & kBlkInside) != 0u);
+    const uint32_t lo = (uint32_t)__builtin_amdgcn_readfirstlane((int)L.r[2 * R].amask.x);
+    const uint32_t hi = (uint32_t)__builtin_amdgcn_readfirstlane((int)L.r[2 * R + 1].amask.x);
+    const uint64_t allow = (uint64_t)hi << 32 | lo;
+    const uint64_t draw = allow & kept & ~culled;
+    const uint64_t cand = allow & ~culled & ~kept;
+    if (lane == 0) L.draw_mask[R] = draw;
+    rs.total += (uint32_t)__popcll(draw);
+    if (lane_of(cand)) ring.code[(rs.head + rs.count + lane_prefix(cand)) & (kBkRing - 1u)] = (uint16_t)(R * 64 + lane);
+    rs.count += (uint32_t)__popcll(cand);
+}
+
+__device__ __forceinline__ void blk_flush(const MeshletCullParams &p, WaveTileLds &L, const PlaneLds &P, const CandRing &ring,
+                                          const StreamRsrc &SR, int lane, RingState &rs, uint32_t n) {
+    __builtin_amdgcn_fence(__ATOMIC_RELEASE, "wavefront");
+    __builtin_amdgcn_wave_barrier();
+    __builtin_amdgcn_fence(__ATOMIC_ACQUIRE, "wavefront");
+    const bool valid = (uint32_t)lane < n;
+    const uint32_t code = valid ? (uint32_t)ring.code[(rs.head + (uint32_t)lane) & (kBkRing - 1u)] : 0u;
+    const uint32_t rid = (code >> 5) & 15u, ml = code & 31u;
+    const uint4 rec = L.r[rid].rec;
+    const uint32_t rel = rec.y + ml - SR.first;
+    const uint32_t i = (valid && ml < rec.z && rel < SR.count) ? rel : kNoOffset >> 4;
+    const auto sp = __builtin_amdgcn_raw_buffer_load_b128(SR.sphere, i << 4, 0, 0);
+    const uint32_t c = __builtin_amdgcn_raw_buffer_load_b32(SR.cone, i << 2, 0, 0);
+    Sphere s;
+    const uint64_t geo = eval_geometry_mask<0>(p, L, P, rid, make_uint4(sp[0], sp[1], sp[2], sp[3]), make_uint4(c, 0u, 0u, 0u), s, true);
+    const uint64_t vis = geo & ballot(valid);
+    if (lane_of(vis)) atomicOr(reinterpret_cast<uint32_t *>(L.draw_mask) + rid, 1u << ml);
+    rs.total += (uint32_t)__popcll(vis);
+    rs.head = (rs.head + n) & (kBkRing - 1u);
+    rs.count -= n;
+}
+
+__global__ __launch_bounds__(kBkWaves * 64, kBkWavesPerSimd) void meshlet_eval_blocks_kernel(const MeshletCullParams p,
+                                                                                            const BlockBound *blk) {
+    __shared__ WaveTileLds lds[kBkWaves][3];
+    __shared__ BlockTileLds blds[kBkWaves][2];
+    __shared__ PlaneLds planes;
+    __shared__ CandRing rings[kBkWaves];
+    __shared__ uint32_t cls_sel[8];
+    const int lane = threadIdx.x & 63, wave = threadIdx.x >> 6;
+    const uint32_t nrec_raw = *reinterpret_cast<const uint32_t *>(p.dispatch_buffer);
+    const uint32_t stride = gridDim.x * kBkWaves, wave_g = blockIdx.x * kBkWaves + wave;
+    const uint32_t cap_tiles = (p.dispatch_capacity + kTileRecords - 1) / kTileRecords;
+    uint4 r0 = setup_load_rec(p, wave_g, wave_g < cap_tiles, p.dispatch_capacity, lane);
+    uint4 r1 = setup_load_rec(p, wave_g + stride, wave_g + stride < cap_tiles, p.dispatch_capacity, lane);
+    uint4 rec2 = setup_load_rec(p, wave_g + 2u * stride, wave_g + 2u * stride < cap_tiles, p.dispatch_capacity, lane);
+    planes_to_lds(p, planes);
+    clear_chunk_sums(p, kBkWaves * 64);
+    if (threadIdx.x < 6) cls_sel[threadIdx.x] = ((alpha_bits(p.ci, threadIdx.x >> 1) >> (threadIdx.x & 1u)) & 1u) ? ~0u : 0u;
+    __syncthreads();
+    const uint32_t nrec = min(nrec_raw, p.dispatch_capacity);
+    const uint32_t ntiles = (nrec + kTileRecords - 1) / kTileRecords;
+    const uint32_t full_rounds = ntiles / stride;
+    const uint32_t dyn_rounds = min(max(full_rounds / 4u, 1u), 3u);
+    const uint32_t n_static = ntiles <= stride ? 0xFFFFFFFFu : max(full_rounds >= dyn_rounds ? full_rounds - dyn_rounds : 0u, 3u);
+    const uint32_t npools = min((uint32_t)kTicketPools, stride);
+    const uint32_t pool = wave_g % npools;
+    uint32_t *ticket_ctr = p.tickets + pool * kTicketStride;
+    uint32_t claims = 0;
+    auto claim = [&]() -> uint32_t {
+        uint32_t raw = claims;
+        if (claims >= n_static) {
+            raw = 0;
+            if (lane == 0) raw = atomicAdd(ticket_ctr, 1u);
+        }
+        claims++;
+        return raw;
+    };
+    auto ticket_tile = [&](uint32_t raw, uint32_t k) -> uint32_t {
+        const uint32_t t = (uint32_t)__builtin_amdgcn_readfirstlane((int)raw);
+        if (k < n_static) return t * stride + wave_g;
+        return t >= 0x08000000u ? 0xFFFFFFFFu : n_static * stride + t * npools + pool;
+    };
+    StreamRsrc SR = {};
+    SR.first = p.ms.first;
+    SR.count = p.ms.count;
+    SR.sphere = __builtin_amdgcn_make_buffer_rsrc(const_cast<uint4 *>(p.ms.sphere + p.ms.first), 0, p.ms.count * 16u, kBufFlags);
+    SR.cone = __builtin_amdgcn_make_buffer_rsrc(const_cast<uint32_t *>(p.ms.cone + p.ms.first), 0, p.ms.count * 4u, kBufFlags);
+    uint32_t w0, w1, w2, tk_raw;
+    {
+        const uint32_t t0 = claim(), t1 = claim(), t2 = claim();
+        tk_raw = claim();
+        w0 = ticket_tile(t0, 0u);
+        w1 = ticket_tile(t1, 1u);
+        w2 = ticket_tile(t2, 2u);
+    }
+    RowRegs<1> qa, qb;
+    {
+        const uint4 none = make_uint4(0u, 0u, 0u, 0u);
+        const uint32_t rl = (uint32_t)lane >> 2;
+        if (!(w0 < ntiles && w0 * kTileRecords + rl < nrec)) r0 = none;
+        if (!(w1 < ntiles && w1 * kTileRecords + rl < nrec)) r1 = none;
+        if (!(w2 < ntiles && w2 * kTileRecords + rl < nrec)) rec2 = none;
+        if ((lane & 3) == 0) lds[wave][0].r[lane >> 2].rec = r0;
+        __builtin_amdgcn_fence(__ATOMIC_RELEASE, "wavefront");
+        __builtin_amdgcn_wave_barrier();
+        __builtin_amdgcn_fence(__ATOMIC_ACQUIRE, "wavefront");
+        const float4 m0 = setup_load_mat(p, r0, lane);
+        const float4 m1 = setup_load_mat(p, r1, lane);
+        const uint32_t c0 = setup_load_cls(p, r0, lane), c1 = setup_load_cls(p, r1, lane);
+        const BoundRegs b0 = blk_load_bound(p, blk, r0, lane), b1 = blk_load_bound(p, blk, r1, lane);
+        blk_row_load<0>(p, lds[wave][0], false, lane, qa, SR);
+        blk_row_load<1>(p, lds[wave][0], false, lane, qb, SR);
+        setup_write_cls(lds[wave][0], cls_sel, r0, c0, lane);
+        setup_write_cls(lds[wave][1], cls_sel, r1, c1, lane);
+        setup_write(p, lds[wave][0], r0, m0, lane);
+        blk_setup(p, lds[wave][0], blds[wave][0], planes, b0, lane);
+        setup_write(p, lds[wave][1], r1, m1, lane);
+        blk_setup(p, lds[wave][1], blds[wave][1], planes, b1, lane);
+    }
+    uint32_t it = 0;
+    const uint32_t prio_rank = blockIdx.x / max(gridDim.x / (uint32_t)kBkWavesPerSimd, 1u);
+    while (w0 < ntiles) {
+        switch ((it + prio_rank) & 3u) {
+        case 0: __builtin_amdgcn_s_setprio(0); break;
+        case 1: __builtin_amdgcn_s_setprio(1); break;
+        case 2: __builtin_amdgcn_s_setprio(2); break;
+        default: __builtin_amdgcn_s_setprio(3); break;
+        }
+        const uint32_t w3 = ticket_tile(tk_raw, claims - 1u);
+        tk_raw = claim();
+        WaveTileLds &L = lds[wave][it % 3];
+        WaveTileLds &Ln = lds[wave][(it + 1) % 3];
+        const BlockTileLds &B = blds[wave][it & 1u];
+        CandRing &ring = rings[wave];
+        RingState rs;
+#define BK_ROW(R, Q)                                                                                                   \
+    if (row_is_sparse(L, R)) blk_row_eval<R>(L, B, ring, lane, Q, rs);                                                 \
+    else rs.total = rows_eval<0, 0, R, 1, true>(p, L, planes, nullptr, lane, Q, rs.total, nullptr);
+#define BK_FLUSH() \
+    while (rs.count >= kBkFlush) blk_flush(p, L, planes, ring, SR, lane, rs, kBkFlush);
+        BK_ROW(0, qa)
+        blk_row_load<2>(p, L, row_is_sparse(L, 2), lane, qa, SR);
+        BK_ROW(1, qb)
+        blk_row_load<3>(p, L, row_is_sparse(L, 3), lane, qb, SR);
+        BK_FLUSH()
+        BK_ROW(2, qa)
+        blk_row_load<4>(p, L, row_is_sparse(L, 4), lane, qa, SR);
+        BK_ROW(3, qb)
+        blk_row_load<5>(p, L, row_is_sparse(L, 5), lane, qb, SR);
+        BK_FLUSH()
+        const float4 mat2 = setup_load_mat(p, rec2, lane);
+        const uint32_t cls2 = setup_load_cls(p, rec2, lane);
+        const BoundRegs bnd2 = blk_load_bound(p, blk, rec2, lane);
+        const uint4 rec3 = setup_load_rec(p, w3, w3 < ntiles, nrec, lane);
+        BK_ROW(4, qa)
+        blk_row_load<6>(p, L, row_is_sparse(L, 6), lane, qa, SR);
+        BK_ROW(5, qb)
+        blk_row_load<7>(p, L, row_is_sparse(L, 7), lane, qb, SR);
+        BK_ROW(6, qa)
+        blk_row_load<0>(p, Ln, row_is_sparse(Ln, 0), lane, qa, SR);
+        BK_ROW(7, qb)
+        blk_row_load<1>(p, Ln, row_is_sparse(Ln, 1), lane, qb, SR);
+#undef BK_ROW
+#undef BK_FLUSH
+        setup_write_cls(lds[wave][(it + 2) % 3], cls_sel, rec2, cls2, lane);
+        setup_write(p, lds[wave][(it + 2) % 3], rec2, mat2, lane);
+        blk_setup(p, lds[wave][(it + 2) % 3], blds[wave][it & 1u], planes, bnd2, lane);
+        while (rs.count > 0u) blk_flush(p, L, planes, ring, SR, lane, rs, min(rs.count, kBkFlush));
+        __builtin_amdgcn_fence(__ATOMIC_RELEASE, "wavefront");
+        __builtin_amdgcn_wave_barrier();
+        __builtin_amdgcn_fence(__ATOMIC_ACQUIRE, "wavefront");
+        if (lane < 2 * (int)kTileRows)
+            p.tile_masks[(size_t)w0 * (2 * kTileRows) + lane] = reinterpret_cast<const uint32_t *>(L.draw_mask)[lane];
+        if (lane == 0) p.tile_counts[w0] = rs.total;
+        w0 = w1;
+        w1 = w2;
+        w2 = w3;
+        rec2 = rec3;
+        it++;
+    }
+}
+
+}
+
+hipError_t launch_meshlet_eval_blocks(const MeshletCullParams &p, const BlockBound *blk, dim3 grid, hipStream_t s) {
+    hipLaunchKernelGGL(meshlet_eval_blocks_kernel, grid, dim3(kBkWaves * 64), 0, s, p, blk);
+    return hipGetLastError();
+}
+
+}
diff --git a/orbit_amd/csrc/meshlet_stream.hip b/orbit_amd/csrc/meshlet_stream.hip
--- a/orbit_amd/csrc/meshlet_stream.hip
+++ b/orbit_amd/csrc/meshlet_stream.hip
@@ -1,3 +1,4 @@
+#include "block_pretest.h"
 #include "kernels.h"
 
 namespace orbit {
@@ -131,7 +132,7 @@
 }
 
 __global__ __launch_bounds__(256) void meshlet_stream_validate_kernel(const OrbitMeshlet *meshlets, const StreamBuildArrays A,
-                                                                      int32_t *status) {
+                                                                      int32_t *status, const BlockBound *blk) {
     for (uint64_t m = A.s_first + (uint64_t)blockIdx.x * 256u + threadIdx.x; m < A.s_end; m += (uint64_t)gridDim.x * 256u) {
         const uint4 *src = reinterpret_cast<const uint4 *>(meshlets + m);
         const uint4 a = src[0], b = src[1], sa = A.sphere[m];
@@ -151,18 +152,68 @@
             const bool link = b.y == pb.y && b.z == pb.z + meshlet_data_words((pb.w >> 16) & 0xFFu, pb.w >> 24);
             same = same && link == (((A.link[m >> 5] >> (m & 31u)) & 1u) != 0u);
         }
+        if (blk != nullptr) {
+            const BlockBound B = blk[m >> 5];
+            if (B.valid != 0u) {
+                const double dx = (double)__uint_as_float(a.x) - B.cx, dy = (double)__uint_as_float(a.y) - B.cy;
+                const double dz = (double)__uint_as_float(a.z) - B.cz, r = (double)__uint_as_float(a.w);
+                const bool inside = dx * dx + dy * dy + dz * dz <= (double)B.rc * B.rc && r <= (double)B.r_max && r >= 0.0;
+                same = same && inside;
+            }
+        }
         if (!same) latch_status(status, ORBIT_E_STALE);
     }
+}
+
+__global__ __launch_bounds__(256) void block_bounds_kernel(const uint4 *sphere, BlockBound *blk, uint64_t block_first,
+                                                           uint64_t block_count, uint64_t s_first, uint64_t s_end) {
+    const uint32_t ml = threadIdx.x & 31u, half = (threadIdx.x >> 5) & 1u;
+    const float inf = __builtin_inff();
+    auto reduce = [](float v, bool want_max) {
+#pragma unroll
+        for (int d = 16; d >= 1; d >>= 1) {
+            const float o = __shfl_xor(v, d, 32);
+            v = want_max ? fmaxf(v, o) : fminf(v, o);
+        }
+        return v;
+    };
+    const uint64_t rounds = (block_count + (uint64_t)gridDim.x * 8u - 1u) / ((uint64_t)gridDim.x * 8u);
+    for (uint64_t it = 0; it < rounds; it++) {
+        const uint64_t k = (it * gridDim.x + blockIdx.x) * 8u + (threadIdx.x >> 5);
+        const uint64_t m = (block_first + k) * 32u + ml;
+        const bool in = k < block_count && m >= s_first && m < s_end;
+        uint4 w = make_uint4(0u, 0u, 0u, 0u);
+        if (in) w = sphere[m];
+        const float x = __uint_as_float(w.x), y = __uint_as_float(w.y), z = __uint_as_float(w.z), r = __uint_as_float(w.w);
+        const bool bad = in && !(__builtin_isfinite(x) && __builtin_isfinite(y) && __builtin_isfinite(z) && __builtin_isfinite(r));
+        const bool finite = (uint32_t)(__ballot(bad) >> (32u * half)) == 0u;
+        const float x0 = reduce(in ? x : inf, false), x1 = reduce(in ? x : -inf, true);
+        const float y0 = reduce(in ? y : inf, false), y1 = reduce(in ? y : -inf, true);
+        const float z0 = reduce(in ? z : inf, false), z1 = reduce(in ? z : -inf, true);
+        const float cx = 0.5f * x0 + 0.5f * x1, cy = 0.5f * y0 + 0.5f * y1, cz = 0.5f * z0 + 0.5f * z1;
+        const float dist = reduce(in ? block_dist(cx, cy, cz, x, y, z) : 0.0f, true);
+        const float r_max = reduce(in ? r : 0.0f, true), r_min = reduce(in ? r : 0.0f, false);
+        if (ml == 0u && k < block_count) blk[block_first + k] = block_bound_finish(cx, cy, cz, dist, r_max, r_min, finite);
+    }
+}
+
+hipError_t launch_block_bounds_build(const uint4 *sphere, BlockBound *blk, uint64_t block_first, uint64_t block_count,
+                                     uint64_t s_first, uint64_t s_end, hipStream_t s) {
+    if (block_count == 0) return hipSuccess;
+    const uint64_t need = (block_count + 7u) / 8u;
+    hipLaunchKernelGGL(block_bounds_kernel, dim3((uint32_t)(need < 8192u ? need : 8192u)), dim3(256), 0, s, sphere, blk,
+                       block_first, block_count, s_first, s_end);
+    return hipGetLastError();
 }
 
 hipError_t launch_meshlet_stream_validate(const OrbitMeshlet *meshlets, const MeshletStreamView &ms,
                                           const OrbitMaterialData *materials, uint32_t material_count, int32_t *status,
-                                          hipStream_t s) {
+                                          hipStream_t s, const BlockBound *blk) {
     if (ms.count == 0) return hipSuccess;
     const uint64_t need = ((uint64_t)ms.count + 255u) / 256u;
     const uint32_t blocks = (uint32_t)(need < 8192u ? need : 8192u);
     hipLaunchKernelGGL(meshlet_stream_validate_kernel, dim3(blocks), dim3(256), 0, s, meshlets,
-                       stream_build_arrays(ms, materials, material_count), status);
+                       stream_build_arrays(ms, materials, material_count), status, blk);
     return hipGetLastError();
 }
 
diff --git a/orbit_amd/engine.py b/orbit_amd/engine.py
--- a/orbit_amd/engine.py
+++ b/orbit_amd/engine.py
@@ -548,6 +548,12 @@
     def meshlet_class_culls(self):
         return int(self._lib.orbit_ctx_meshlet_class_culls(self._ctx))
 
+    def block_culls(self):
+        return int(self._lib.orbit_ctx_block_culls(self._ctx))
+
+    def set_block_cull(self, enable):
+        _lib.check(self._lib.orbit_ctx_set_block_cull(self._ctx, 1 if enable else 0), self._ctx)
+
     def exchange_list(self, local_list, rank, world, out_buffers, ctrl_buffers, out_capacity, header_bytes, stride,
                       stream=None):
         outs = (C.c_void_p * world)(*[_ptr(b) for b in out_buffers])
diff --git a/orbit_amd/host/orbit_host_c.cpp b/orbit_amd/host/orbit_host_c.cpp
--- a/orbit_amd/host/orbit_host_c.cpp
+++ b/orbit_amd/host/orbit_host_c.cpp
@@ -10,6 +10,7 @@
 #include "orbit_gltf.hpp"
 #include "orbit_raster.hpp"
 #include "orbit_scene.hpp"
+#include "../csrc/block_pretest.h"
 
 using namespace orbit;
 using namespace orbit::passes;
@@ -661,4 +662,23 @@
     scale[0] = t.scale.x, scale[1] = t.scale.y, scale[2] = t.scale.z;
 }
 
-}
+void orbit_host_block_bounds(const float *spheres, uint64_t count, void *out) {
+    orbit::BlockBound *o = static_cast<orbit::BlockBound *>(out);
+    for (uint64_t b = 0; b * 32u < count; b++) o[b] = orbit::block_bound_of(spheres + 128u * b, (uint32_t)std::min<uint64_t>(32u, count - 32u * b));
+}
+
+uint32_t orbit_host_block_pretest(const float m[16], int32_t affine, float scale, const void *bound, const float *planes,
+                                  uint32_t n_planes, float ratio, const uint32_t *cones, uint64_t count, uint8_t *verdicts) {
+    orbit::BlockBound in;
+    memcpy(&in, bound, sizeof(in));
+    const orbit::BlockBound b = orbit::block_bound_unpack(in.cx, in.cy, in.cz, in.packed);
+    const orbit::BlockRecord r = orbit::block_record_setup(m, affine != 0, scale, b, true, planes, n_planes, ratio < 0.0f ? ORBIT_BLK_RATIO : ratio);
+    for (uint64_t i = 0; i < count; i++) {
+        uint32_t v = (r.flags & orbit::kBlkSparse) ? orbit::block_pretest(r, cones[i]) : 0u;
+        if (v == 2u && (r.flags & orbit::kBlkInside)) v |= 4u;
+        verdicts[i] = (uint8_t)v;
+    }
+    return r.flags;
+}
+
+}
diff --git a/orbit_amd/host/orbit_host_c.h b/orbit_amd/host/orbit_host_c.h
--- a/orbit_amd/host/orbit_host_c.h
+++ b/orbit_amd/host/orbit_host_c.h
@@ -211,6 +211,9 @@
                                        uint64_t index_count, uint64_t target_index_count, uint32_t *out,
                                        uint64_t capacity, uint64_t *needed);
 void orbit_host_transform_from_mat4(const float matrix[16], float position[3], float orientation[4], float scale[3]);
+void orbit_host_block_bounds(const float *spheres, uint64_t count, void *out);
+uint32_t orbit_host_block_pretest(const float m[16], int32_t affine, float scale, const void *bound, const float *planes,
+                                  uint32_t n_planes, float ratio, const uint32_t *cones, uint64_t count, uint8_t *verdicts);
 #ifdef __cplusplus
 }
 #endif
```

Measured after the change: 209.4 billion (median of 6 runs). 7.2% higher.
